# JosephCatrambone/aruco3

Measured on AMD Instinct MI355X. Metric: frames/sec at 1920x1080 ARUCO dict, higher is better.
Workload: dtype u8

## Files before the change

aruco3_amd/_lib.py:

```python
import ctypes as C
from pathlib import Path

import numpy as np

import os

_HERE = Path(__file__).resolve().parent
LIB_PATH = Path(os.environ["A3_HIP_LIB"]).resolve() if os.environ.get("A3_HIP_LIB") else _HERE / "libaruco3_hip.so"

OK, ERR_INVALID, ERR_HIP, ERR_CAPACITY, ERR_INTERNAL, ERR_NO_DEVICE, ERR_LIMIT = 0, -1, -2, -3, -4, -5, -6
FMT_RGB8, FMT_RGBA8, FMT_L8, FMT_BGRA8 = 0, 1, 2, 3
FMT_YUYV8, FMT_UYVY8 = 5, 6
MEM_HOST, MEM_DEVICE = 0, 1
PROFILE_OFF, PROFILE_STAGES, PROFILE_THRESHOLD_ONLY, PROFILE_THRESHOLD_SAMPLED = 0, 1, 2, 3
STAGE_THRESHOLD, STAGE_CONTOUR, STAGE_DECODE = 0, 1, 2
STEP_WHOLE, STEP_DECODE_DEFERRED, STEP_HELD_RELEASED_BY_LAST, STEP_HELD_RELEASED_EARLY, STEP_BURST_LAST, STEP_HELD = 0, 1, 2, 3, 4, 5
REFINE_NONE, REFINE_SUBPIX, REFINE_EDGES = 0, 1, 2
BOARD_NONE, BOARD_OK = 0, 1
BOARD_MAX_MARKERS = 1024
DIST_NONE, DIST_RATIONAL = 0, 1
DIST_FISHEYE = 3
CHARUCO_MAX_CORNERS = 2048
CHARUCO_NO_ADJ = 0xFFFFFFFF
CALIB_FIX_PRINCIPAL_POINT, CALIB_ZERO_TANGENT_DIST, CALIB_FIX_K3, CALIB_RATIONAL_MODEL, CALIB_USE_INTRINSIC_GUESS = 1, 2, 4, 8, 16
CALIB_OK, CALIB_TOO_FEW, CALIB_NO_INIT, CALIB_NOT_FINITE = 1, 2, 3, 4
CALIB_VIEW_USED, CALIB_VIEW_TOO_FEW_POINTS, CALIB_VIEW_DEGENERATE = 1, 2, 3
CALIB_MAX_POINTS, CALIB_MAX_VIEWS, CALIB_MAX_CAMERAS, CALIB_MAX_CALL_VIEWS = 4096, 4096, 1024, 65536
FISHEYE_FIX_PRINCIPAL_POINT, FISHEYE_FIX_K1, FISHEYE_FIX_K2, FISHEYE_FIX_K3, FISHEYE_FIX_K4, FISHEYE_USE_INTRINSIC_GUESS = 1, 2, 4, 8, 16, 32
FISHEYE_START_MAX_R = 4.0
RIG_USE_EXTRINSIC_GUESS, RIG_FIX_EXTRINSICS = 1, 2
RIG_OK, RIG_NOT_CONNECTED, RIG_NOT_FINITE = 1, 2, 3
RIG_OBS_USED, RIG_OBS_TOO_FEW_POINTS, RIG_OBS_DEGENERATE = 1, 2, 3
RIG_FRAME_USED, RIG_FRAME_UNUSED = 1, 2
RIG_MAX_CAMERAS, RIG_MAX_FRAMES, RIG_MAX_RIGS, RIG_MAX_CALL_FRAMES, RIG_MAX_CALL_OBSERVATIONS = 8, 4096, 1024, 65536, 262144
HANDEYE_USE_GUESS, HANDEYE_FIX_X = 1, 2
HANDEYE_OK, HANDEYE_TOO_FEW_FRAMES, HANDEYE_NO_MOTION, HANDEYE_NOT_FINITE = 1, 2, 3, 4
HANDEYE_FRAME_USED, HANDEYE_FRAME_TOO_FEW_POINTS, HANDEYE_FRAME_DEGENERATE = 1, 2, 3
HANDEYE_MAX_FRAMES, HANDEYE_MAX_PROBLEMS, HANDEYE_MAX_CALL_FRAMES = 256, 1024, 65536
HANDEYE_MIN_PIVOT_RATIO = 1e-4
MAP_USE_GUESS, MAP_FIX_MAP = 1, 2
MAP_OK, MAP_NOT_CONNECTED, MAP_NOT_FINITE = 1, 2, 3
MAP_MARKER_USED, MAP_MARKER_UNSEEN, MAP_MARKER_UNREACHED = 1, 2, 3
MAP_FRAME_USED, MAP_FRAME_UNUSED = 1, 2
MAP_OBS_USED, MAP_OBS_DEGENERATE, MAP_OBS_UNREACHED = 1, 2, 3
MAP_MAX_MARKERS, MAP_MAX_FRAMES, MAP_MAX_MAPS, MAP_MAX_CALL_FRAMES, MAP_MAX_CALL_OBSERVATIONS, MAP_START_OBSERVATIONS = 128, 4096, 1024, 65536, 262144, 8
STEP_NAMES = {0: "whole", 1: "decode_deferred", 2: "held_released_by_last", 3: "held_released_early", 4: "burst_last", 5: "held"}

SYMBOLS = [
    "a3_abi_version", "a3_default_config", "a3_create", "a3_destroy", "a3_last_error", "a3_set_stream", "a3_get_stream", "a3_set_pool_limits",
    "a3_get_tau", "a3_order_after", "a3_set_debug_taps", "a3_detect_batch", "a3_detect_batch_pose", "a3_detect_batch_submit", "a3_detect_batch_collect", "a3_detect_batch_pose_submit", "a3_detect_batch_pose_collect",
    "a3_host_alloc", "a3_host_free", "a3_host_register", "a3_host_unregister", "a3_get_stats", "a3_synth_render", "a3_download_grey", "a3_download_thresholded",
    "a3_candidate_count", "a3_download_candidates", "a3_download_homographies", "a3_estimate_pose", "a3_estimate_pose_normalized",
    "a3_find_nearest", "a3_calculate_tau", "a3_set_profiling", "a3_get_profile",
    "a3_contour_count", "a3_download_contours", "a3_detection_record_bytes", "a3_pack_detections",
    "a3_default_refine_config", "a3_set_corner_refinement", "a3_get_refined_corners", "a3_refine_corners",
    "a3_set_board", "a3_get_board_poses", "a3_estimate_board_pose",
    "a3_default_recover_config", "a3_set_board_recovery", "a3_get_board_recovery", "a3_get_recovered_counts", "a3_recover_markers",
    "a3_default_distortion", "a3_set_distortion", "a3_get_undistorted_corners", "a3_undistort_points",
    "a3_default_charuco_config", "a3_set_charuco", "a3_get_charuco_corners", "a3_get_charuco_poses", "a3_interpolate_charuco",
    "a3_calibrate_cameras", "a3_calibrate_fisheye_cameras", "a3_calibrate_rigs", "a3_calibrate_hand_eyes", "a3_build_marker_maps",
    "a3_default_rectify", "a3_rectify_frames", "a3_set_rectification", "a3_get_rectification",
    "a3_reduce_frames", "a3_set_reduction", "a3_get_reduction",
]
CAND_DTYPE = np.dtype([("start_key", "<u4"), ("xy", "<u2", (8,))])
PROJ_DTYPE = np.dtype([("inv", "<f4", (9,)), ("ok", "<i4")])
CONTOUR_DTYPE = np.dtype([("frame", "<u4"), ("start_key", "<u4"), ("point_base", "<u4"), ("n", "<u4")])
INTERNAL_SYMBOLS = ["a3_debug_set_overlap", "a3_debug_build_flags", "a3_debug_spin", "a3_debug_set_hold", "a3_debug_set_jump_rounds", "a3_debug_launch_threshold", "a3_debug_kernel_time", "a3_selftest_ieee", "a3_debug_clockwise", "a3_debug_rotate_bits", "a3_debug_discard_too_near", "a3_debug_inject_candidates", "a3_debug_sample_frames", "a3_debug_frame_candidates", "a3_debug_contour_quads"]


class A3Error(RuntimeError):
    def __init__(self, code, message):
        super().__init__(f"aruco3_hip error {code}: {message}")
        self.code = code


class Config(C.Structure):
    _fields_ = [
        ("threshold_window", C.c_uint32),
        ("contour_simplification_epsilon", C.c_double),
        ("min_side_length_factor", C.c_float),
        ("min_corner_separation_factor", C.c_float),
        ("homography_sample_size", C.c_uint32),
        ("filter_high_bit_errors", C.c_uint8),
    ]


class MarkerRec(C.Structure):
    _fields_ = [
        ("frame", C.c_uint32),
        ("id", C.c_uint32),
        ("code", C.c_uint64),
        ("corners", C.c_uint32 * 8),
        ("hamming_distance", C.c_uint8),
        ("rotation", C.c_uint8),
        ("candidate_index", C.c_uint16),
    ]


MARKER_DTYPE = np.dtype([("frame", "<u4"), ("id", "<u4"), ("code", "<u8"), ("corners", "<u4", (8,)), ("hamming_distance", "u1"),
                         ("rotation", "u1"), ("candidate_index", "<u2")], align=True)
assert MARKER_DTYPE.itemsize == C.sizeof(MarkerRec) == 56


class PoseRec(C.Structure):
    _fields_ = [("error", C.c_float), ("rotation", C.c_float * 9), ("translation", C.c_float * 3)]


class Intrinsics(C.Structure):
    _fields_ = [("image_width", C.c_uint32), ("image_height", C.c_uint32), ("focal_x", C.c_float), ("focal_y", C.c_float),
                ("principal_x", C.c_float), ("principal_y", C.c_float)]


class RefineConfig(C.Structure):
    _fields_ = [("method", C.c_uint32), ("win_half", C.c_uint32), ("relative_win", C.c_float), ("max_iterations", C.c_uint32),
                ("min_shift", C.c_float)]


class BoardPoseRec(C.Structure):
    _fields_ = [("status", C.c_uint32), ("markers_used", C.c_uint32), ("markers_rejected", C.c_uint32), ("iterations", C.c_uint32),
                ("rms_px", C.c_float), ("alt_rms_px", C.c_float), ("rotation", C.c_float * 9), ("translation", C.c_float * 3)]


class RecoverConfig(C.Structure):
    _fields_ = [("mode", C.c_uint32), ("min_markers", C.c_uint32), ("max_distance_px", C.c_float), ("max_hamming", C.c_uint8),
                ("reserved", C.c_uint8 * 3)]


RECOVER_NO_BITS = 255


class DistortionRec(C.Structure):
    _fields_ = [("model", C.c_uint32), ("iterations", C.c_uint32), ("k1", C.c_float), ("k2", C.c_float), ("p1", C.c_float),
                ("p2", C.c_float), ("k3", C.c_float), ("k4", C.c_float), ("k5", C.c_float), ("k6", C.c_float),
                ("max_residual_px", C.c_float)]


class CharucoConfig(C.Structure):
    _fields_ = [("min_markers", C.c_uint32), ("refine", C.c_uint32), ("win_half", C.c_uint32), ("relative_win", C.c_float),
                ("max_iterations", C.c_uint32), ("min_shift", C.c_float)]


CHARUCO_CORNER_DTYPE = np.dtype([("frame", "<u4"), ("id", "<u4"), ("x", "<f4"), ("y", "<f4"), ("interp_x", "<f4"), ("interp_y", "<f4"),
                                 ("markers_used", "<u4"), ("window", "<u4")])
CHARUCO_POSE_DTYPE = np.dtype([("status", "<u4"), ("corners_used", "<u4"), ("iterations", "<u4"), ("reserved", "<u4"), ("rms_px", "<f4"),
                               ("alt_rms_px", "<f4"), ("rotation", "<f4", (9,)), ("translation", "<f4", (3,))])
BOARD_POSE_DTYPE = np.dtype([("status", "<u4"), ("markers_used", "<u4"), ("markers_rejected", "<u4"), ("iterations", "<u4"),
                             ("rms_px", "<f4"), ("alt_rms_px", "<f4"), ("rotation", "<f4", (9,)), ("translation", "<f4", (3,))])


class CalibCamera(C.Structure):
# ... 123 lines not shown
    def as_dict(self):
        d = {k: int(getattr(self, k)) for k, _ in self._fields_}
        d["released_others"] = (d["stepping"] >> 8) & 0xFF
        d["reruns"] = (d["stepping"] >> 16) & 0xFF
        d["stepping"] = STEP_NAMES.get(d["stepping"] & 0xFF, d["stepping"] & 0xFF)
        return d


_lib = None


def load():
    global _lib
    if _lib is not None:
        return _lib
    try:
        import torch
    except ImportError:
        pass
    if not LIB_PATH.exists():
        raise ImportError(f"{LIB_PATH} is missing: build the HIP library first (python -c 'import __graft_entry__ as g; g.build()'). "
                          "aruco3_amd has no CPU fallback.")
    L = C.CDLL(str(LIB_PATH))
    vp, u8p, u32p, u64p, f32p, f64p = C.c_void_p, C.POINTER(C.c_uint8), C.POINTER(C.c_uint32), C.POINTER(C.c_uint64), C.POINTER(C.c_float), C.POINTER(C.c_double)
    L.a3_abi_version.restype = C.c_int
    L.a3_default_config.restype = None
    L.a3_default_config.argtypes = [C.POINTER(Config)]
    L.a3_create.restype = C.c_int
    L.a3_create.argtypes = [C.c_int, C.POINTER(Config), u64p, C.c_size_t, C.c_uint8, C.c_uint8, C.POINTER(vp)]
    L.a3_destroy.restype = None
    L.a3_destroy.argtypes = [vp]
    L.a3_last_error.restype = C.c_char_p
    L.a3_last_error.argtypes = [vp]
    L.a3_set_stream.restype = C.c_int
    L.a3_set_stream.argtypes = [vp, vp]
    L.a3_get_stream.restype = C.c_int
    L.a3_get_stream.argtypes = [vp, C.POINTER(vp)]
    L.a3_detect_batch_pose_submit.restype = C.c_int
    L.a3_detect_batch_pose_submit.argtypes = [vp, vp, C.c_int, C.c_int, C.c_uint32, C.c_uint32, C.c_size_t, C.c_size_t, C.c_uint32, C.c_float,
                                              C.POINTER(Intrinsics), C.c_size_t]
    L.a3_detect_batch_pose_collect.restype = C.c_int
    L.a3_detect_batch_pose_collect.argtypes = [vp, vp, vp, C.c_size_t, u32p, C.POINTER(C.c_size_t)]
    L.a3_order_after.restype = C.c_int
    L.a3_order_after.argtypes = [vp, vp]
    L.a3_host_alloc.restype = C.c_int
    L.a3_host_alloc.argtypes = [C.c_size_t, C.POINTER(vp)]
    L.a3_host_free.restype = C.c_int
    L.a3_host_free.argtypes = [vp]
    L.a3_host_register.restype = C.c_int
    L.a3_host_register.argtypes = [vp, C.c_size_t]
    L.a3_host_unregister.restype = C.c_int
    L.a3_host_unregister.argtypes = [vp]
    L.a3_set_pool_limits.restype = C.c_int
    L.a3_set_pool_limits.argtypes = [vp, C.c_uint64, C.c_uint64]
    L.a3_get_tau.restype = C.c_int
    L.a3_get_tau.argtypes = [vp, u8p]
    L.a3_set_debug_taps.restype = C.c_int
    L.a3_set_debug_taps.argtypes = [vp, C.c_int]
    L.a3_detect_batch.restype = C.c_int
    L.a3_detect_batch.argtypes = [vp, vp, C.c_int, C.c_int, C.c_uint32, C.c_uint32, C.c_size_t, C.c_size_t, C.c_uint32, vp, C.c_size_t, u32p,
                                  C.POINTER(C.c_size_t)]
    L.a3_detect_batch_submit.restype = C.c_int
    L.a3_detect_batch_submit.argtypes = [vp, vp, C.c_int, C.c_int, C.c_uint32, C.c_uint32, C.c_size_t, C.c_size_t, C.c_uint32, C.c_size_t]
    L.a3_detect_batch_collect.restype = C.c_int
    L.a3_detect_batch_collect.argtypes = [vp, vp, C.c_size_t, u32p, C.POINTER(C.c_size_t)]
    L.a3_detect_batch_pose.restype = C.c_int
    L.a3_detect_batch_pose.argtypes = [vp, vp, C.c_int, C.c_int, C.c_uint32, C.c_uint32, C.c_size_t, C.c_size_t, C.c_uint32, C.c_float,
                                       C.POINTER(Intrinsics), vp, vp, C.c_size_t, u32p, C.POINTER(C.c_size_t)]
    L.a3_synth_render.restype = C.c_int
    L.a3_synth_render.argtypes = [C.c_int, vp, vp, C.c_uint32, vp, C.c_uint32, C.c_uint32, C.c_uint32, C.c_int, C.c_float, C.c_float, C.c_int,
                                  vp, C.c_size_t, C.c_size_t]
    if hasattr(L, "a3_debug_set_overlap"):
        L.a3_debug_set_overlap.restype = C.c_int
        L.a3_debug_set_overlap.argtypes = [C.c_int]
    if hasattr(L, "a3_debug_launch_threshold"):
        L.a3_debug_launch_threshold.restype = C.c_int
        L.a3_debug_launch_threshold.argtypes = [vp, vp, C.c_int, C.c_uint32, C.c_uint32, C.c_uint32]
    if hasattr(L, "a3_debug_set_hold"):
        L.a3_debug_set_hold.restype = C.c_int
        L.a3_debug_set_hold.argtypes = [C.c_int]
    if hasattr(L, "a3_debug_set_jump_rounds"):
        L.a3_debug_set_jump_rounds.restype = C.c_int
        L.a3_debug_set_jump_rounds.argtypes = [C.c_int]
    if hasattr(L, "a3_debug_spin"):
        L.a3_debug_spin.restype = C.c_int
        L.a3_debug_spin.argtypes = [vp, C.c_int, C.c_int, C.c_int]
    if hasattr(L, "a3_debug_build_flags"):
        L.a3_debug_build_flags.restype = C.c_int
        L.a3_debug_build_flags.argtypes = []
    L.a3_debug_kernel_time.restype = C.c_int
    L.a3_debug_kernel_time.argtypes = [vp, C.c_int, C.c_int, C.c_int, C.POINTER(C.c_float)]
    L.a3_get_stats.restype = C.c_int
    L.a3_get_stats.argtypes = [vp, C.POINTER(Stats)]
    L.a3_download_grey.restype = C.c_int
    L.a3_download_grey.argtypes = [vp, C.c_uint32, u8p]
    L.a3_download_thresholded.restype = C.c_int
    L.a3_download_thresholded.argtypes = [vp, C.c_uint32, u8p]
    L.a3_candidate_count.restype = C.c_int
    L.a3_candidate_count.argtypes = [vp, C.c_uint32, u32p, u32p]
    L.a3_download_candidates.restype = C.c_int
    L.a3_download_candidates.argtypes = [vp, C.c_uint32, C.c_int, u32p, C.c_size_t]
    L.a3_download_homographies.restype = C.c_int
    L.a3_download_homographies.argtypes = [vp, C.c_uint32, u8p, u8p, u64p, C.POINTER(C.c_int32), C.c_size_t]
    L.a3_estimate_pose.restype = C.c_int
    L.a3_estimate_pose.argtypes = [vp, u32p, C.c_size_t, C.c_float, C.POINTER(Intrinsics), C.c_uint32, C.c_uint32, C.POINTER(PoseRec)]
    L.a3_estimate_pose_normalized.restype = C.c_int
    L.a3_estimate_pose_normalized.argtypes = [vp, f32p, C.c_size_t, C.c_float, C.POINTER(PoseRec)]
    L.a3_find_nearest.restype = C.c_int
    L.a3_find_nearest.argtypes = [vp, u64p, C.c_size_t, u32p, u8p]
    L.a3_calculate_tau.restype = C.c_int
    L.a3_calculate_tau.argtypes = [C.c_int, u64p, C.c_size_t, u8p]
    L.a3_set_profiling.restype = C.c_int
    L.a3_set_profiling.argtypes = [vp, C.c_int]
    L.a3_get_profile.restype = C.c_int
    L.a3_get_profile.argtypes = [vp, C.c_int, f64p, u64p, C.c_int]
    L.a3_selftest_ieee.restype = C.c_int
    L.a3_selftest_ieee.argtypes = [vp, f64p, f64p, C.c_size_t, f64p, f64p, f32p, f32p]
    L.a3_contour_count.restype = C.c_int
    L.a3_contour_count.argtypes = [vp, C.c_uint32, u32p, u64p]
    L.a3_download_contours.restype = C.c_int
    L.a3_download_contours.argtypes = [vp, C.c_uint32, u32p, u32p, u32p, C.c_size_t, C.c_size_t]
    L.a3_detection_record_bytes.restype = C.c_size_t
    L.a3_detection_record_bytes.argtypes = [C.c_uint32, C.c_int]
    L.a3_pack_detections.restype = C.c_int
    L.a3_pack_detections.argtypes = [vp, C.c_uint32, C.c_uint32, C.c_int, vp, C.c_size_t]
    L.a3_debug_clockwise.restype = C.c_int
    L.a3_debug_clockwise.argtypes = [vp, C.POINTER(C.c_int32), C.c_size_t, C.POINTER(C.c_int32)]
    L.a3_debug_rotate_bits.restype = C.c_int
    L.a3_debug_rotate_bits.argtypes = [vp, u8p, C.c_uint32, C.c_uint32, u8p]
    L.a3_debug_inject_candidates.restype = C.c_int
    L.a3_debug_inject_candidates.argtypes = [vp, u32p, C.c_size_t]
    if hasattr(L, "a3_debug_sample_frames"):
        L.a3_debug_sample_frames.restype = C.c_int
        L.a3_debug_sample_frames.argtypes = [vp, C.c_int]
    if hasattr(L, "a3_refine_corners"):
        L.a3_default_refine_config.restype = None
        L.a3_default_refine_config.argtypes = [C.POINTER(RefineConfig)]
        L.a3_set_corner_refinement.restype = C.c_int
        L.a3_set_corner_refinement.argtypes = [vp, C.POINTER(RefineConfig)]
        L.a3_get_refined_corners.restype = C.c_int
        L.a3_get_refined_corners.argtypes = [vp, f32p, C.c_size_t, C.POINTER(C.c_size_t)]
        L.a3_refine_corners.restype = C.c_int
        L.a3_refine_corners.argtypes = [vp, vp, C.c_int, C.c_int, C.c_uint32, C.c_uint32, C.c_size_t, f32p, f32p, C.c_size_t]
    if hasattr(L, "a3_set_board"):
        L.a3_set_board.restype = C.c_int
        L.a3_set_board.argtypes = [vp, u32p, f32p, C.c_size_t]
        L.a3_get_board_poses.restype = C.c_int
        L.a3_get_board_poses.argtypes = [vp, vp, C.c_size_t, C.POINTER(C.c_size_t)]
        L.a3_estimate_board_pose.restype = C.c_int
        L.a3_estimate_board_pose.argtypes = [vp, u32p, f32p, C.c_size_t, C.POINTER(Intrinsics), C.c_uint32, C.c_uint32, C.POINTER(BoardPoseRec)]
    if hasattr(L, "a3_set_board_recovery"):
        u64p, u8p = C.POINTER(C.c_uint64), C.POINTER(C.c_uint8)
        L.a3_default_recover_config.restype = C.c_int
        L.a3_default_recover_config.argtypes = [vp, C.POINTER(RecoverConfig)]
        L.a3_set_board_recovery.restype = C.c_int
        L.a3_set_board_recovery.argtypes = [vp, C.POINTER(RecoverConfig)]
        L.a3_get_board_recovery.restype = C.c_int
        L.a3_get_board_recovery.argtypes = [vp, C.POINTER(RecoverConfig)]
        L.a3_get_recovered_counts.restype = C.c_int
        L.a3_get_recovered_counts.argtypes = [vp, u32p, C.c_size_t]
        L.a3_recover_markers.restype = C.c_int
        L.a3_recover_markers.argtypes = [vp, u32p, u32p, C.c_size_t, u32p, u64p, u8p, C.c_size_t, C.POINTER(RecoverConfig), vp, C.c_size_t,
                                         C.POINTER(C.c_size_t)]
    if hasattr(L, "a3_set_distortion"):
        L.a3_default_distortion.restype = None
        L.a3_default_distortion.argtypes = [C.POINTER(DistortionRec)]
# ... 675 lines not shown
```

aruco3_amd/csrc/a3_api.hip:

```cpp
#include <algorithm>
#include <atomic>
#include <cmath>
#include <chrono>
#include <cstddef>
#include <cstdio>
#include <cstring>
#include <mutex>
#include <string>
#include <vector>

#include "a3_common.h"
#include "a3_format.h"
#include "a3_internal.h"
#include "a3_launch.h"
#include "a3_readback.h"
#include "a3_rectify_check.h"
#include "a3_reduce_check.h"
#include "a3_solve_check.h"

using namespace a3;

namespace {

thread_local std::string g_create_error;

constexpr uint32_t kPatchCapMin = 32768, kPatchCapMax = 1u << 20;

struct DevBuf {
    void* p = nullptr;
    size_t cap = 0;
    hipError_t ensure(size_t bytes) {
        if (bytes <= cap) return hipSuccess;
        if (p) { hipError_t e = hipFree(p); p = nullptr; cap = 0; if (e != hipSuccess) return e; }
        hipError_t e = hipMalloc(&p, bytes);
        if (e == hipSuccess) cap = bytes;
        return e;
    }
    void release() { if (p) (void)hipFree(p); p = nullptr; cap = 0; }
    template <typename T> T* as() const { return reinterpret_cast<T*>(p); }
};

template <typename T> struct Seg { size_t off, n; };
struct Layout {
    DevBuf& buf;
    hipStream_t stream;
    size_t end = 0;
    template <typename T> Seg<T> add(size_t n, size_t elem = sizeof(T)) {
        const size_t off = (end + 255) & ~(size_t)255;
        end = off + n * elem;
        return {off, n};
    }
    hipError_t ensure() { return buf.ensure((end + 255) & ~(size_t)255); }
    template <typename T> T* at(Seg<T> s) const { return reinterpret_cast<T*>(buf.as<uint8_t>() + s.off); }
    template <typename T> hipError_t upload(Seg<T> s, const T* src, size_t n) const {
        return n ? hipMemcpyAsync(at(s), src, n * sizeof(T), hipMemcpyHostToDevice, stream) : hipSuccess;
    }
    template <typename T> hipError_t download(Seg<T> s, T* dst) const {
        return dst ? hipMemcpyAsync(dst, at(s), s.n * sizeof(T), hipMemcpyDeviceToHost, stream) : hipSuccess;
    }
    template <typename T> hipError_t zero_from(Seg<T> s) const { return hipMemsetAsync(at(s), 0, end - s.off, stream); }
};

struct Batch {
    const uint8_t* pixels = nullptr; int fmt = 0;
    uint32_t W = 0, H = 0, n = 0;
    size_t row_stride = 0, frame_stride = 0, out_cap = 0;
    bool want_pose = false, pose_has_intr = false;
    float pose_size_mm = 0.0f;
    a3_intrinsics pose_intr{};
    a3_refine_config refine{};
    bool refined = false;
    bool board = false;
    a3_distortion dist{};
    bool undist = false;
    bool charuco = false;
    a3_charuco_config charuco_cfg{};
    uint32_t charuco_nc = 0, charuco_guess = 0;
    bool recover = false;
    a3_recover_config recover_cfg{};
    uint32_t recover_slots = 0, recover_cap = 0;
    uint32_t sides = 0;
    bool has(int kind) const { return (sides >> kind & 1u) != 0; }
    enum class Plane { None, Rectified, Reduced } plane = Plane::None;
    PixelSrc frames{};
    uint32_t frames_W = 0, frames_H = 0;
    a3_rectify rect_r{};
    uint32_t reduce_f = 0;
    bool taps = false;
    bool sample_frames = false;
    int profiling = 0, profile_every = 1;
    int prof = 0;
    bool need_grey = false;
    bool grey_src = false;
    uint32_t max_cand = 0, patch_cap = 0, marker_cap = 0, guess = 0;
    bool active = false, device_plan = false;
    size_t n_chunks = 0;
    Readback rb;
    uint64_t chunk0_darts = 0;
    int rounds_max = 0;
    PixelSrc src{};
};

}

struct a3_ctx {
    int device = 0;
    hipStream_t own_stream = nullptr, stream = nullptr;
    hipEvent_t ev_in = nullptr;
    hipEvent_t ev_contours = nullptr, ev_k1 = nullptr, ev_k1_done = nullptr, ev_gate = nullptr;
    bool gates_declared = false;
    bool rest_held = false;
    int held_rc = 0;
    bool back_deferred = false;
    int back_rc = 0;
    bool allow_defer = false;
    int batch_mode = 0;
    std::atomic<uint32_t> stepping{0};
    uint32_t released_others = 0;
    uint32_t reruns = 0;
    a3_config cfg{};
    uint8_t num_bits = 0, tau = 0;
    uint32_t n_codes = 0, mark_size = 0;
    std::string err;

    uint64_t max_darts = kMaxDartsDefault;
    BatchHints hints;
    uint32_t dbg_nd = 0, dbg_frames = 0, dbg_chunks = 0;
    PixelSrc dbg_src{};
    std::vector<CandRec> inject;
    bool inject_armed = false;
    uint32_t inject_count = 0;
    Batch batch;
    bool pending_trivial = false;
    bool busy() const { return batch.active || pending_trivial; }
    bool debug_taps = false;
    bool debug_sample_frames = false;
    uint32_t patch_cap = 0;
    bool grey_valid = false;
    bool contours_valid = false;
    uint32_t tap_contours = 0; uint64_t tap_points = 0;
    bool markers_valid = false;
    uint32_t last_n = 0, last_max_per_frame = 0;
    int profiling = 0;
    int profile_every = 1;
    uint32_t batch_seq = 0;
    hipEvent_t ev[6] = {nullptr, nullptr, nullptr, nullptr, nullptr, nullptr};
    double prof_ms[A3_STAGE_COUNT] = {0, 0, 0};
    uint64_t prof_n[A3_STAGE_COUNT] = {0, 0, 0};
    a3_stats stats{};

    uint32_t W = 0, H = 0, frames = 0;

    DevBuf dict, in, grey, bin, frame_darts, frame_darts_dev, frame_base, pix_base, tile_darts;
    DevBuf d_xy, d_succ, fin, t_cur, t_next;
    DevBuf leader_list, leader_keep, entry_list, es_a, es_b;
    DevBuf contours, cyc_start_off, points;
    DevBuf cands, pre_xy, fin_xy, fin_count, work, outs, proj, patches, cand_big;
    DevBuf zero_blk;
    a3_marker* markers_ptr = nullptr;
    unsigned long long* frame_darts_ptr = nullptr;
    BatchScratch* head = nullptr; DeviceCounters* counters = nullptr; uint32_t* per_frame = nullptr; uint32_t* frame_cursor = nullptr; uint32_t* cand_count = nullptr;
    uint32_t last_marker_total = 0;
    DevBuf tmp_a, tmp_b, tmp_c, tmp_d;
    DevBuf hsum;
    DevBuf wtab;
    DevBuf pose_buf;
    void* side_dev[kSideKinds] = {};
    std::vector<uint8_t> side_h[kSideKinds];
    bool side_valid[kSideKinds] = {};
    a3_refine_config refine{};
    a3_refine_config refine_prm_cfg{};
    std::vector<float> refine_prm;
    DevBuf refined_buf;
    std::vector<uint32_t> board_ids;
    std::vector<uint8_t> board_slots;
    uint64_t board_version = 0, board_dev_version = 0;
    std::vector<uint16_t> board_slot_up;
    std::vector<uint8_t> board_slots_up;
    DevBuf board_slot_of, board_slot_rec, board_buf;
    a3_recover_config recover{};
    uint64_t recover_ids_version = 0;
    std::vector<uint32_t> recover_ids_up;
    DevBuf recover_ids, recover_counts, recover_det, recover_tmp;
    a3_distortion dist{};
    DevBuf undist_buf;
    a3_charuco_config charuco_cfg{};
    std::vector<uint32_t> charuco_tab_h;
    uint32_t charuco_nc = 0;
    uint64_t charuco_version = 0, charuco_dev_version = 0;
    std::vector<uint32_t> charuco_tab_up;
    a3_charuco_config charuco_prm_cfg{};
    std::vector<float> charuco_prm;
    DevBuf charuco_tab, charuco_tmp, charuco_buf, charuco_und, charuco_pose_buf;
    std::vector<a3_charuco_corner> h_charuco;
    bool charuco_valid = false;
    DevBuf solve_in, solve_scratch, solve_big, solve_out;
    DevBuf rect_in, rect_out;
    a3_rectify rect{};
    bool rect_on = false;
    a3_reduction reduction{};
    DevBuf plane;
    uint32_t last_charuco_total = 0;
    void* pinned = nullptr;
    size_t pinned_cap = 0;
    void* pinned_counts = nullptr;
    size_t pinned_counts_cap = 0;
    std::vector<uint32_t> h_cand_pre, h_cand_fin;
    bool counts_valid = false;
};

namespace {

int fail(a3_ctx* c, int code, const char* what, hipError_t e = hipSuccess) {
    char buf[512];
    if (e != hipSuccess) snprintf(buf, sizeof buf, "%s: %s", what, hipGetErrorString(e));
    else snprintf(buf, sizeof buf, "%s", what);
    if (c) c->err = buf; else g_create_error = buf;
    return code;
}

#define A3_HIP(call)                                                        \
    do {                                                                    \
        hipError_t e_ = (call);                                             \
        if (e_ != hipSuccess) return fail(ctx, A3_ERR_HIP, #call, e_);      \
    } while (0)

inline void spin_pause() {
#if defined(__x86_64__) || defined(__i386__)
    __builtin_ia32_pause();
#endif
}
constexpr auto kSpinBudget = std::chrono::milliseconds(2);

hipError_t wait_stream(hipStream_t st) {
    const auto t0 = std::chrono::steady_clock::now();
    for (;;) {
        const hipError_t e = hipStreamQuery(st);
        if (e != hipErrorNotReady) return e;
        if (std::chrono::steady_clock::now() - t0 > kSpinBudget) return hipStreamSynchronize(st);
        spin_pause();
    }
}

hipError_t wait_event(hipEvent_t ev, hipStream_t st) {
    (void)hipStreamQuery(st);
// ... 295 lines not shown
    const uint32_t n = b.n;
    const ZeroLayout z = zero_layout(1, n, n, b.marker_cap);
    A3_HIP(ctx->tile_darts.ensure(tile_darts_bytes(b.W, b.H, n)));
    A3_HIP(ctx->zero_blk.ensure(z.total));
    if (ctx->frame_darts_dev.cap < (size_t)n * 8) {
        A3_HIP(ctx->frame_darts_dev.ensure((size_t)n * 8));
        A3_HIP(hipMemsetAsync(ctx->frame_darts_dev.p, 0, ctx->frame_darts_dev.cap, st));
    }
    A3_HIP(ctx->frame_base.ensure((size_t)(n + 1) * 4));
    if (int rc = ensure_dart_pool(ctx, pool_darts_of(ctx->max_darts, cap_d, 1))) return rc;
    A3_HIP(ctx->pix_base.ensure((size_t)n * b.W * b.H * 4));
    A3_HIP(ctx->contours.ensure((size_t)ctx->hints.max_contours * sizeof(ContourRec)));
    A3_HIP(ctx->cyc_start_off.ensure((size_t)ctx->hints.max_contours * 4));
    A3_HIP(ctx->points.ensure(ctx->hints.max_points * 4));
    return ensure_back_buffers(ctx, b, z.head_bytes);
}


int enqueue_front(a3_ctx* ctx, Batch& b, bool held) {
    hipStream_t st = ctx->stream;
    const uint32_t n = b.n, W = b.W, H = b.H;
    const size_t npx = (size_t)W * H;
    const uint32_t kMaxCand = ctx->hints.max_cand;
    const bool big_window = threshold_writes_grey_plane(ctx->cfg.threshold_window);
    b.need_grey = b.taps || big_window;
    b.grey_src = big_window || (b.taps && !b.sample_frames);
    if (b.need_grey) A3_HIP(ctx->grey.ensure(npx * n));
    ctx->grey_valid = b.need_grey;
    if (big_window) A3_HIP(ctx->hsum.ensure(npx * n * 2));
    const size_t bits_per_frame = (size_t)words_per_row(W) * 8 * H;
    A3_HIP(ctx->bin.ensure(bits_per_frame * n));
    A3_HIP(ctx->frame_darts.ensure((size_t)n * 8));
    A3_HIP(ctx->cands.ensure((size_t)n * kMaxCand * sizeof(CandRec)));
    A3_HIP(ctx->pre_xy.ensure((size_t)n * kMaxCand * 16));
    A3_HIP(ctx->fin_xy.ensure((size_t)n * kMaxCand * 16));
    A3_HIP(ctx->fin_count.ensure((size_t)n * 4));
    A3_HIP(ctx->work.ensure((size_t)n * kMaxCand * 4));
    if (kMaxCand > frame_cand_lds_slots()) A3_HIP(ctx->cand_big.ensure((size_t)n * kMaxCand * 4));
    A3_HIP(ctx->outs.ensure((size_t)n * kMaxCand * decode_out_bytes()));
    A3_HIP(ctx->proj.ensure((size_t)n * kMaxCand * proj_rec_bytes()));
    b.max_cand = kMaxCand;
    b.marker_cap = marker_cap_of(kMaxCand, n, b.out_cap);
    b.guess = marker_guess_of(ctx->last_marker_total, b.marker_cap);
    b.patch_cap = (uint32_t)std::min<uint64_t>(kPatchCapMax, std::max<uint64_t>(kPatchCapMin, (uint64_t)n * kMaxCand));
    if (b.taps) { A3_HIP(ctx->patches.ensure((size_t)b.patch_cap * ctx->cfg.homography_sample_size * ctx->cfg.homography_sample_size)); ctx->patch_cap = b.patch_cap; }
    ctx->W = W; ctx->H = H; ctx->frames = n;
    ctx->stats = a3_stats{};
    ctx->contours_valid = false; ctx->markers_valid = false; ctx->side_valid[kSidePoses] = false;

    b.prof = b.profiling == 1 && (ctx->batch_seq++ % (uint32_t)b.profile_every) != 0 ? 0 : b.profiling;
    const PixelSrc& fr = b.frames;
    if (b.plane == Batch::Plane::Rectified)
        A3_HIP(launch_rectify_grey(st, {.src = fr.base, .src_row = (size_t)fr.row_stride, .src_frame = (size_t)fr.frame_stride, .n_frames = n, .fmt = fr.fmt,
                                        .r = &b.rect_r, .grey = ctx->plane.as<uint8_t>()}));
    if (b.plane == Batch::Plane::Reduced)
        A3_HIP(launch_reduce_frames(st, {.src = fr.base, .src_row = (size_t)fr.row_stride, .src_frame = (size_t)fr.frame_stride, .n_frames = n, .fmt = fr.fmt,
                                         .W = b.frames_W, .H = b.frames_H, .factor = b.reduce_f, .dst = ctx->plane.as<uint8_t>(), .dst_row = W,
                                         .dst_frame = npx}));
    if (b.prof) A3_HIP(hipEventRecord(ctx->ev[0], st));
    A3_HIP(launch_grey_threshold(st, {.pixels = b.pixels, .fmt = b.fmt, .row_stride = b.row_stride, .frame_stride = b.frame_stride, .W = (int)W, .H = (int)H,
                                      .n = n, .radius = ctx->cfg.threshold_window, .grey = b.need_grey ? ctx->grey.as<uint8_t>() : nullptr,
                                      .bits = ctx->bin.as<uint64_t>(), .hsum_tmp = big_window ? ctx->hsum.as<uint16_t>() : nullptr}));
    if (b.prof) A3_HIP(hipEventRecord(ctx->ev[1], st));
    if (!held) return A3_OK;
    A3_HIP(hipEventRecord(ctx->ev_k1_done, st));
    const uint64_t cap_d = device_plan_capacity(ctx->hints, ctx->max_darts, n, W, H);
    if (cap_d == 0) return fail(ctx, A3_ERR_INTERNAL, "a chain was held back for a batch that needs a host-side plan");
    return ensure_chain_buffers(ctx, st, b, cap_d);
}

ContourChunk contour_chunk(const a3_ctx* ctx) {
    ContourChunk c;
    c.W = (int)ctx->W; c.H = (int)ctx->H; c.batch_frames = ctx->frames;
    c.bits = ctx->bin.as<uint64_t>(); c.tile_darts = ctx->tile_darts.as<uint32_t>(); c.pix_base = ctx->pix_base.as<uint32_t>();
    c.d_rec = ctx->d_xy.as<uint64_t>(); c.d_succ = ctx->d_succ.as<uint32_t>();
    c.entry_list = ctx->entry_list.as<uint32_t>(); c.es_a = ctx->es_a.p; c.es_b = ctx->es_b.p; c.fin = ctx->fin.p;
    c.leader_count = ctx->head->leader_count; c.entry_count = ctx->head->entry_count;
    c.leader_list = ctx->leader_list.as<uint32_t>(); c.leader_keep = ctx->leader_keep.as<uint32_t>();
    c.t_cur = ctx->t_cur.as<uint64_t>(); c.t_next = ctx->t_next.as<uint64_t>();
    c.contours = ctx->contours.as<ContourRec>(); c.cyc_start_off = ctx->cyc_start_off.as<uint32_t>(); c.points = ctx->points.as<uint32_t>();
    c.max_contours = ctx->hints.max_contours; c.max_points = ctx->hints.max_points;
    c.cands = ctx->cands.as<CandRec>(); c.cand_count = ctx->cand_count;
    c.err_flags = &ctx->head->err_flags;
    return c;
}

int enqueue_chain(a3_ctx* ctx, Batch& b, bool defer_locked) {
    hipStream_t st = ctx->stream;
    const uint32_t n = b.n, W = b.W, H = b.H;
    const int rel_mode = defer_locked ? 0 : release_mode();
    const size_t npx = (size_t)W * H;
    const uint32_t minwh = W < H ? W : H;
    const uint32_t min_edge_length = (uint32_t)((float)minwh * ctx->cfg.min_side_length_factor);
    const uint32_t kMaxCand = b.max_cand;
    bool released = false;
    auto release_waiting = [&]() -> int {
        if (released) return A3_OK;
        std::lock_guard<std::mutex> lk(g_defer_mu);
        bool any = false;
        for (a3_ctx* o : g_deferred) any |= (o != ctx && o->device == ctx->device);
        if (!any) return A3_OK;
        released = true;
        A3_HIP(hipEventRecord(ctx->ev_k1, st));
        const std::vector<a3_ctx*> list = g_deferred;
        for (a3_ctx* o : list)
            if (o != ctx && o->device == ctx->device)
                if (int rc = flush_deferred_locked(o, ctx->ev_k1)) { ctx->err = "deferred decode of another context: " + o->err; return rc; }
        return A3_OK;
    };
    if (rel_mode == 1) { if (int rc = release_waiting()) return rc; }

    const uint64_t cap_d = device_plan_capacity(ctx->hints, ctx->max_darts, n, W, H);
    const bool device_plan = cap_d != 0;
    size_t head_bytes = 0, head_off = 0;
    void* zero_p = nullptr; size_t zero_bytes = 0;
    auto layout_zero_block = [&](size_t n_chunks, uint32_t chunk_frames, bool launch) -> hipError_t {
        const ZeroLayout zl = zero_layout(n_chunks, chunk_frames, n, b.marker_cap);
        head_bytes = zl.head_bytes; head_off = zl.head_off;
        const hipError_t e = ctx->zero_blk.ensure(zl.total);
        if (e != hipSuccess) return e;
        uint8_t* z = ctx->zero_blk.as<uint8_t>();
        ctx->frame_cursor = reinterpret_cast<uint32_t*>(z);
        ctx->cand_count = ctx->frame_cursor + chunk_frames;
        ctx->head = reinterpret_cast<BatchScratch*>(z + head_off);
        ctx->counters = reinterpret_cast<DeviceCounters*>(ctx->head + 1);
        ctx->per_frame = reinterpret_cast<uint32_t*>(ctx->counters + n_chunks);
        ctx->markers_ptr = reinterpret_cast<a3_marker*>(z + head_off + head_bytes);
        zero_p = z; zero_bytes = (head_off + head_bytes + 15) & ~(size_t)15;
        return launch ? launch_zero(st, zero_p, zero_bytes) : hipSuccess;
    };
    std::vector<Chunk> chunks;
    std::vector<uint64_t> fd;
    if (device_plan) {
        if (int rc = ensure_chain_buffers(ctx, st, b, cap_d)) return rc;
        chunks.push_back(Chunk{0, n, cap_d, (uint32_t)std::min<uint64_t>(cap_d, 0xFFFFFFFFu)});
        A3_HIP(layout_zero_block(1, n, false));
        ctx->frame_darts_ptr = ctx->frame_darts_dev.as<unsigned long long>();
    } else {
        A3_HIP(ctx->tile_darts.ensure(tile_darts_bytes(W, H, n)));
        ctx->frame_darts_ptr = ctx->frame_darts.as<unsigned long long>();
        A3_HIP(hipMemsetAsync(ctx->frame_darts.p, 0, (size_t)n * 8, st));
    }
    DartCountLaunch count{.bits = ctx->bin.as<uint64_t>(), .W = (int)W, .H = (int)H, .n_frames = n, .frame_darts = ctx->frame_darts_ptr,
                          .tile_darts = ctx->tile_darts.as<uint32_t>(), .plan_cap = cap_d};
    if (device_plan) { count.frame_base = ctx->frame_base.as<uint32_t>(); count.plan = &ctx->head->plan; count.zero_p = zero_p; count.zero_bytes = zero_bytes; }
    A3_HIP(launch_dart_count(st, count));
    const uint32_t* n_live = device_plan ? &ctx->head->plan.darts : nullptr;
    uint32_t max_chunk_frames = n;
    if (!device_plan) {
        if (int rc = ensure_pinned(ctx, std::max<size_t>((size_t)n * 8, 1 << 16))) return rc;
        A3_HIP(hipMemcpyAsync(ctx->pinned, ctx->frame_darts.p, (size_t)n * 8, hipMemcpyDeviceToHost, st));
        A3_HIP(wait_stream(st));
        fd.assign((uint64_t*)ctx->pinned, (uint64_t*)ctx->pinned + n);
        chunks.resize(n);
        const ChunkSplit split = split_chunks(fd.data(), n, ctx->max_darts, kMaxChunkFrames, chunks.data());
        ctx->stats.darts += split.total_darts;
        if (split.refused) return fail(ctx, A3_ERR_LIMIT, "a frame needs more contour-graph nodes than 32-bit indices allow");
        ctx->max_darts = split.max_darts;
        chunks.resize(split.n_chunks);
        max_chunk_frames = split.max_chunk_frames;
        if (int rc = ensure_dart_pool(ctx, pool_darts_of(ctx->max_darts, split.max_chunk_darts, chunks.size()))) return rc;
        A3_HIP(ctx->pix_base.ensure((size_t)max_chunk_frames * npx * 4));
        A3_HIP(ctx->frame_base.ensure((size_t)(max_chunk_frames + 1) * 4 * chunks.size()));
        A3_HIP(layout_zero_block(chunks.size(), max_chunk_frames, true));
        A3_HIP(ctx->contours.ensure((size_t)ctx->hints.max_contours * sizeof(ContourRec)));
        A3_HIP(ctx->cyc_start_off.ensure((size_t)ctx->hints.max_contours * 4));
        A3_HIP(ctx->points.ensure(ctx->hints.max_points * 4));
        const size_t stride = max_chunk_frames + 1, n_bases = stride * chunks.size();
        if (int rc = ensure_pinned(ctx, (size_t)n * 8 + n_bases * 4 + (1 << 16))) return rc;
        uint32_t* h_bases = reinterpret_cast<uint32_t*>((uint8_t*)ctx->pinned + (size_t)n * 8);
        for (size_t ci = 0; ci < chunks.size(); ci++) chunk_frame_bases(fd.data(), chunks[ci], (uint32_t)stride, h_bases + ci * stride);
        A3_HIP(hipMemcpyAsync(ctx->frame_base.p, h_bases, n_bases * 4, hipMemcpyHostToDevice, st));
    }
    ctx->stats.chunks = (uint32_t)chunks.size();

    ContourChunk cc = contour_chunk(ctx);
    cc.n_live = n_live;
    cc.resolve_iters = ctx->hints.resolve_full_ttl > 0 ? ctx->hints.resolve_iters_hint : 0;
    cc.inline_resolve_W = ctx->hints.resolve_full_ttl > 0 ? 0 : (int)W;
    cc.min_edge_length = min_edge_length;
    cc.eps_factor = ctx->cfg.contour_simplification_epsilon;
    cc.keep_all = b.taps;
    cc.max_cand = kMaxCand;
    int rounds_max = 0;
    for (size_t ci = 0; ci < chunks.size(); ci++) {
        const Chunk& c = chunks[ci];
        const uint32_t nd = (uint32_t)c.darts;
        if (nd == 0) continue;
        if (ci > 0) {
            A3_HIP(hipMemsetAsync(cc.leader_count, 0, sizeof(BatchScratch::leader_count) + sizeof(BatchScratch::entry_count), st));
            A3_HIP(hipMemsetAsync(ctx->frame_cursor, 0, (size_t)c.count * 4, st));
        }
        cc.first_frame = c.first; cc.n_frames = c.count; cc.n_darts = nd;
        cc.frame_base = ctx->frame_base.as<uint32_t>() + ci * (max_chunk_frames + 1);
        cc.ctr = ctx->counters + ci;
        A3_HIP(launch_dart_build(st, cc));
        const int rounds = chunk_rounds(c.max_frame_darts, ctx->hints.jump_rounds_hint, g_jump_rounds_cap.load(std::memory_order_relaxed));
        rounds_max = std::max(rounds_max, rounds);
        cc.max_rounds = rounds;
        cc.frame_entries = ctx->hints.entry_global_ttl > 0 ? nullptr : ctx->frame_cursor;
        const bool dense_graph = (uint64_t)nd * 10u >= (uint64_t)c.count * npx;
        cc.dead_count = (b.taps || !dense_graph) ? nullptr : ctx->head->dead_count;
        cc.phase = 1;
        A3_HIP(launch_rank_cycles(st, cc));
        if (rel_mode == 2) { if (int rc = release_waiting()) return rc; }
        ctx->dbg_nd = nd; ctx->dbg_frames = c.count; ctx->dbg_chunks = (uint32_t)chunks.size();
        cc.phase = 2;
        A3_HIP(launch_rank_cycles(st, cc));
        A3_HIP(launch_resolve(st, cc));
        A3_HIP(launch_select_scatter(st, cc));
        A3_HIP(launch_contour_quads(st, cc));
    }
    if (rel_mode != 0) { if (int rc = release_waiting()) return rc; }
    if (b.prof >= 2) A3_HIP(hipEventRecord(ctx->ev[2], st));

    b.src = b.grey_src ? PixelSrc{ctx->grey.as<uint8_t>(), W, (unsigned long long)npx, kFmtGreyPlane}
                        : PixelSrc{b.pixels, b.row_stride, b.frame_stride, b.fmt};
    ctx->dbg_src = b.src;
    if (int rc = ensure_back_buffers(ctx, b, head_bytes)) return rc;
    b.device_plan = device_plan; b.n_chunks = chunks.size(); b.chunk0_darts = chunks.empty() ? 0 : chunks[0].darts;
    b.rounds_max = rounds_max;
    ctx->counts_valid = false;
    if (ctx->allow_defer && !defer_locked && b.profiling < 2 && ctx->batch_mode != 0) {
        A3_HIP(hipEventRecord(ctx->ev_contours, st));
        std::lock_guard<std::mutex> lk(g_defer_mu);
        ctx->back_deferred = true;
        ctx->back_rc = 0;
        ctx->stepping = A3_STEP_DECODE_DEFERRED;
        g_deferred.push_back(ctx);
    } else if (int rc = enqueue_back(ctx, st, b)) return rc;
    b.active = true;
    return A3_OK;
}

int enqueue_batch(a3_ctx* ctx) {
    ctx->stepping = A3_STEP_WHOLE;
    if (int rc = enqueue_front(ctx, ctx->batch, false)) return rc;
    return enqueue_chain(ctx, ctx->batch, false);
}

int finish_batch(a3_ctx* ctx, a3_marker* out, a3_pose* poses, size_t out_cap, uint32_t* per_frame_count, size_t* out_n) {
    Batch& b = ctx->batch;
    if (!b.active) return fail(ctx, A3_ERR_INVALID, "no batch was submitted");
    {
        std::lock_guard<std::mutex> lk(g_defer_mu);
        (void)flush_held_locked(ctx, nullptr);
        if (const int rc = ctx->held_rc) { ctx->held_rc = 0; b.active = false; return rc; }
    }
    b.active = false;
    hipStream_t st = ctx->stream;
    const size_t n_chunks = b.n_chunks;
    const uint32_t guess = b.guess, n = b.n;
    uint8_t* hp = (uint8_t*)ctx->pinned;
    Readback rb = b.rb;
    {
        std::lock_guard<std::mutex> lk(g_defer_mu);
        if (int rc = flush_deferred_locked(ctx, nullptr)) return rc;
        if (const int rc = ctx->back_rc) { ctx->back_rc = 0; return rc; }
    }
    A3_HIP(wait_event(ctx->ev[4], st));
    const BatchScratch& hs = *reinterpret_cast<const BatchScratch*>(hp);
    const DeviceCounters* hc = reinterpret_cast<const DeviceCounters*>(&hs + 1);
    const size_t slot_bytes = sizeof(CandRec) + 16 + 16 + 4 + decode_out_bytes() + proj_rec_bytes();
    const Verdict v = batch_verdict(hs, hc, {.n = n, .W = b.W, .H = b.H, .device_plan = b.device_plan, .n_chunks = n_chunks, .chunk0_darts = b.chunk0_darts,
                                             .rounds_max = b.rounds_max, .out_cap = out_cap, .lds_slots = frame_cand_lds_slots(), .slot_bytes = slot_bytes},
                                    ctx->hints);
    if (b.device_plan && !hs.plan.overflow) ctx->stats.darts = ctx->dbg_nd = v.darts;
    ctx->stats.contours_traced = v.contours_traced; ctx->stats.contours_materialised = v.contours_materialised;
    ctx->stats.jump_rounds = v.jump_rounds; ctx->stats.resolve_iterations = v.resolve_iterations;
    if (v.action == Verdict::Fail) return fail(ctx, v.code, v.message);
    if (v.action == Verdict::GrowCands) {
        const size_t had = ctx->cands.cap + ctx->pre_xy.cap + ctx->fin_xy.cap + ctx->work.cap + ctx->cand_big.cap + ctx->outs.cap + ctx->proj.cap;
        const size_t want = (size_t)n * v.next_cand * v.slot_bytes;
        size_t free_b = 0, total_b = 0;
        if (want > had && hipMemGetInfo(&free_b, &total_b) == hipSuccess && want - had > free_b)
            return fail(ctx, A3_ERR_LIMIT, "candidate tables of this batch do not fit the device (every frame gets the fullest frame's table): fewer frames per call");
        ctx->hints.max_cand = v.next_cand;
    }
    if (v.action != Verdict::Deliver) return 1;
    const uint32_t total = v.total, n_work = v.n_work, n_pre = v.n_pre;
    const uint32_t* hpf = reinterpret_cast<const uint32_t*>(hc + n_chunks);
    if (per_frame_count) memcpy(per_frame_count, hpf, (size_t)n * 4);
    uint32_t max_per_frame = 0;
    for (uint32_t f = 0; f < n; f++) max_per_frame = std::max(max_per_frame, hpf[f]);
    for (int k = 0; k < kSideKinds; k++)
        if (b.has(k) && kSides[k].per_frame) ctx->side_h[k].assign(at<uint8_t>(hp, rb.side[k]), at<uint8_t>(hp, rb.side[k]) + rb.side[k].bytes);
    if (b.charuco) {
        uint32_t charuco_total = 0;
        memcpy(&charuco_total, at<uint8_t>(hp, rb.charuco_total), 4);
        ctx->h_charuco.resize(charuco_total);
        const size_t staged = std::min<uint32_t>(charuco_total, b.charuco_guess);
        if (staged) memcpy(ctx->h_charuco.data(), at<uint8_t>(hp, rb.charuco), staged * sizeof(a3_charuco_corner));
        if (charuco_total > staged) {
            A3_HIP(hipMemcpyAsync(ctx->h_charuco.data() + staged, ctx->charuco_buf.as<a3_charuco_corner>() + staged,
                                  (charuco_total - staged) * sizeof(a3_charuco_corner), hipMemcpyDeviceToHost, st));
            A3_HIP(hipStreamSynchronize(ctx->stream));
        }
        ctx->last_charuco_total = charuco_total;
    }
    if (total > guess) {
        rb = refetch_layout(readback_shape(b, 0), total);
        if (int rc = ensure_pinned(ctx, pinned_bytes(rb))) return rc;
        hp = (uint8_t*)ctx->pinned;
        auto fetch = [&](const Span& to, const void* from) { return hipMemcpyAsync(at<uint8_t>(hp, to), from, to.bytes, hipMemcpyDeviceToHost, st); };
        A3_HIP(fetch(rb.markers, ctx->markers_ptr));
        for (int k = 0; k < kSideKinds; k++)
            if (b.has(k) && !kSides[k].per_frame) A3_HIP(fetch(rb.side[k], ctx->side_dev[k]));
        A3_HIP(hipStreamSynchronize(ctx->stream));
    }
    if (total) {
        memcpy(out, at<a3_marker>(hp, rb.markers), (size_t)total * sizeof(a3_marker));
        if (b.want_pose && poses) memcpy(poses, at<a3_pose>(hp, rb.side[kSidePoses]), (size_t)total * 2 * sizeof(a3_pose));
    }
    for (int k = 0; k < kSideKinds; k++) {
        const uint8_t* const h = at<uint8_t>(hp, rb.side[k]);
        if (b.has(k) && !kSides[k].per_frame && kSides[k].kept) ctx->side_h[k].assign(h, h + (size_t)total * kSides[k].rec);
        ctx->side_valid[k] = b.has(k);
    }
    ctx->charuco_valid = b.charuco;
    if (b.taps) {
        const uint32_t* hc32 = reinterpret_cast<const uint32_t*>(ctx->pinned_counts);
        ctx->h_cand_pre.assign(hc32, hc32 + n);
        ctx->h_cand_fin.assign(hc32 + n, hc32 + 2 * (size_t)n);
        for (auto& v : ctx->h_cand_pre) v = std::min(v, ctx->hints.max_cand);
        ctx->counts_valid = true;
    }
    ctx->last_marker_total = total;
    *out_n = total;
    ctx->stats.markers = total;
    ctx->stats.candidates = n_work;
    ctx->stats.candidates_pre = n_pre;
    ctx->markers_valid = true; ctx->last_n = n; ctx->last_max_per_frame = max_per_frame;
    ctx->contours_valid = b.taps && n_chunks == 1;
    if (ctx->contours_valid) { ctx->tap_contours = v.tap_contours; ctx->tap_points = v.tap_points; }
    if (b.prof >= 1) {
        float ms;
        A3_HIP(hipEventElapsedTime(&ms, ctx->ev[0], ctx->ev[1])); ctx->prof_ms[A3_STAGE_THRESHOLD] += ms; ctx->prof_n[A3_STAGE_THRESHOLD]++;
        if (b.prof >= 2) {
            A3_HIP(hipEventElapsedTime(&ms, ctx->ev[1], ctx->ev[2])); ctx->prof_ms[A3_STAGE_CONTOUR] += ms; ctx->prof_n[A3_STAGE_CONTOUR]++;
            A3_HIP(hipEventElapsedTime(&ms, ctx->ev[2], ctx->ev[3])); ctx->prof_ms[A3_STAGE_DECODE] += ms; ctx->prof_n[A3_STAGE_DECODE]++;
        }
    }
    return A3_OK;
}

int run_batch(a3_ctx* ctx, a3_marker* out, a3_pose* poses, size_t out_cap, uint32_t* per_frame_count, size_t* out_n) {
    if (int rc = enqueue_batch(ctx)) return rc;
    return finish_batch(ctx, out, poses, out_cap, per_frame_count, out_n);
}

// ... 534 lines not shown
        } else if (kernel == 1) {
            cc.dbg = dbg ? dbg : 5;
            A3_HIP(launch_dart_build(st, cc));
        } else if (kernel == 2) {
            cc.dbg = dbg ? dbg : 11;
            A3_HIP(launch_rank_cycles(st, cc));
        } else if (kernel == 3 || kernel == 4) {
            if (kernel == 4) {
                const size_t sweep = std::min<size_t>(ctx->pix_base.cap & ~(size_t)15, (size_t)512 << 20);
                if (sweep) A3_HIP(launch_zero(st, ctx->pix_base.p, sweep));
                A3_HIP(hipEventRecord(e0, st));
            }
            DecodeStage dec = decode_stage(ctx);
            dec.src = ctx->dbg_src; dec.W = cc.W; dec.H = cc.H; dec.max_cand = ctx->hints.max_cand; dec.few = ctx->frames <= 64u; dec.grid_blocks = 4096;
            dec.per_frame = nullptr;
            dec.projection = dbg >= 0; dec.variant = dbg < 0 ? -dbg : dbg;
            A3_HIP(launch_decode(st, dec));
        } else if (kernel == 6) {
            const Batch& b = ctx->batch;
            if (!b.refined || b.plane == Batch::Plane::Reduced || (dbg != A3_REFINE_SUBPIX && dbg != A3_REFINE_EDGES))
                return fail(ctx, A3_ERR_INVALID, "kernel 6: needs a preceding unreduced batch with corner refinement, and dbg = the method to time");
            a3_refine_config rc = b.refine;
            rc.method = (uint32_t)dbg;
            const RefineLaunch rl{.src = ctx->dbg_src, .W = (uint32_t)cc.W, .H = (uint32_t)cc.H, .markers = ctx->markers_ptr, .n_dev = &ctx->head->marker_total,
                                  .n = b.marker_cap, .params = refine_params_for(ctx, rc), .out = ctx->refined_buf.as<float>()};
            A3_HIP(dbg == A3_REFINE_EDGES ? launch_refine_edges(st, rl) : launch_refine_corners(st, rl));
        } else return fail(ctx, A3_ERR_INVALID, "kernel: 0 dart_count, 1 dart_assign, 2 local_contract, 3 decode, 4 decode on cold frames, 6 corner refinement");
        A3_HIP(hipEventRecord(e1, st));
        A3_HIP(hipStreamSynchronize(ctx->stream));
        float ms = 0;
        A3_HIP(hipEventElapsedTime(&ms, e0, e1));
        total += ms;
    }
    *avg_ms = (float)(total / reps);
    return A3_OK;
}

int a3_debug_set_overlap(int mode) {
    if (mode < -1 || mode > 2) return A3_ERR_INVALID;
    std::lock_guard<std::mutex> lk(g_defer_mu);
    if (!g_held.empty() || !g_deferred.empty()) return A3_ERR_INVALID;
    g_overlap_force.store(mode, std::memory_order_relaxed);
    return A3_OK;
}

int a3_debug_spin(void* hip_stream, int workgroups, int threads, int usec) {
    if (workgroups < 1 || workgroups > 1024 || threads < 64 || threads > 512 || threads % 64 || usec < 1 || usec > 100000) return A3_ERR_INVALID;
    static uint32_t* sink = nullptr;
    static std::mutex mu;
    {
        std::lock_guard<std::mutex> lk(mu);
        if (!sink) {
            if (hipMalloc(&sink, 4096 * 4) != hipSuccess) return A3_ERR_HIP;
            if (hipMemset(sink, 0, 4096 * 4) != hipSuccess) return A3_ERR_HIP;
        }
    }
    return launch_spin(reinterpret_cast<hipStream_t>(hip_stream), workgroups, threads, usec, sink) == hipSuccess ? A3_OK : A3_ERR_HIP;
}

int a3_debug_build_flags(void) { return 0; }

int a3_debug_launch_threshold(a3_ctx* ctx, const void* pixels_device, int fmt, uint32_t width, uint32_t height, uint32_t n_frames) {
    if (!ctx || !pixels_device || n_frames == 0) return A3_ERR_INVALID;
    A3_HIP(hipSetDevice(ctx->device));
    if (int rc = need_stream(ctx)) return rc;
    if (!format_valid(fmt) || format_width_error(fmt, width)) return A3_ERR_INVALID;
    const size_t bpp = format_bpp(fmt);
    if (threshold_writes_grey_plane(ctx->cfg.threshold_window))
        return fail(ctx, A3_ERR_INVALID, "a3_debug_launch_threshold: this threshold_window / frame layout takes the separable path, which needs a grey plane");
    A3_HIP(ctx->bin.ensure((size_t)words_per_row(width) * 8 * height * n_frames));
    A3_HIP(launch_grey_threshold(ctx->stream, {.pixels = reinterpret_cast<const uint8_t*>(pixels_device), .fmt = fmt, .row_stride = (size_t)width * bpp,
                                               .frame_stride = (size_t)width * bpp * height, .W = (int)width, .H = (int)height, .n = n_frames,
                                               .radius = ctx->cfg.threshold_window, .bits = ctx->bin.as<uint64_t>()}));
    return A3_OK;
}

int a3_debug_set_hold(int on) {
    std::lock_guard<std::mutex> lk(g_defer_mu);
    if (!g_held.empty()) return A3_ERR_INVALID;
    g_hold_rests = on != 0;
    return A3_OK;
}

int a3_debug_set_jump_rounds(int rounds) {
    if (rounds < 0 || rounds > 32) return A3_ERR_INVALID;
    g_jump_rounds_cap.store(rounds, std::memory_order_relaxed);
    return A3_OK;
}

int a3_synth_render(int device, void* hip_stream, const a3_synth_frame* frames, uint32_t n_frames, const a3_synth_marker* markers,
                    uint32_t n_markers, uint32_t width, uint32_t height, int paper, float black, float white, int supersample,
                    void* out_rgb_device, size_t row_stride, size_t frame_stride) {
    if (!frames || !out_rgb_device || (n_markers && !markers) || supersample < 1 || supersample > 8) return A3_ERR_INVALID;
    if (n_frames == 0 || width == 0 || height == 0) return A3_OK;
    if (row_stride == 0) row_stride = (size_t)width * 3;
    if (frame_stride == 0) frame_stride = row_stride * height;
    if (row_stride < (size_t)width * 3 || frame_stride < row_stride * (height - 1) + (size_t)width * 3 || height > 65535 || n_frames > 65535)
        return A3_ERR_INVALID;
    for (uint32_t f = 0; f < n_frames; f++)
        if ((uint64_t)frames[f].first_marker + frames[f].n_markers > n_markers) return A3_ERR_INVALID;
    for (uint32_t m = 0; m < n_markers; m++)
        if (markers[m].n == 0 || markers[m].n > 11) return A3_ERR_INVALID;
    if (hipSetDevice(device) != hipSuccess) return A3_ERR_NO_DEVICE;
    hipStream_t st = reinterpret_cast<hipStream_t>(hip_stream);
    a3_synth_frame* d_frames = nullptr; a3_synth_marker* d_markers = nullptr;
    hipError_t e = hipMalloc(&d_frames, sizeof(a3_synth_frame) * n_frames);
    if (e == hipSuccess && n_markers) e = hipMalloc(&d_markers, sizeof(a3_synth_marker) * n_markers);
    if (e == hipSuccess) e = hipMemcpyAsync(d_frames, frames, sizeof(a3_synth_frame) * n_frames, hipMemcpyHostToDevice, st);
    if (e == hipSuccess && n_markers) e = hipMemcpyAsync(d_markers, markers, sizeof(a3_synth_marker) * n_markers, hipMemcpyHostToDevice, st);
    if (e == hipSuccess) e = launch_synth_render(st, {.frames = d_frames, .n_frames = n_frames, .markers = d_markers, .W = width, .H = height, .paper = paper,
                                                      .black = black, .white = white, .supersample = supersample,
                                                      .out = reinterpret_cast<uint8_t*>(out_rgb_device), .row_stride = row_stride, .frame_stride = frame_stride});
    if (e == hipSuccess) e = hipStreamSynchronize(st);
    if (d_frames) (void)hipFree(d_frames);
    if (d_markers) (void)hipFree(d_markers);
    return e == hipSuccess ? A3_OK : A3_ERR_HIP;
}

int a3_get_stats(const a3_ctx* ctx, a3_stats* stats) {
    if (!ctx || !stats) return A3_ERR_INVALID;
    *stats = ctx->stats;
    stats->stepping = ctx->stepping | (std::min(ctx->released_others, 255u) << 8) | (std::min(ctx->reruns, 255u) << 16);
    return A3_OK;
}

static int download_plane(a3_ctx* ctx, const DevBuf& buf, uint32_t frame, uint8_t* dst) {
    if (!ctx || !dst) return A3_ERR_INVALID;
    if (frame >= ctx->frames) return fail(ctx, A3_ERR_INVALID, "frame index outside the last batch");
    const size_t npx = (size_t)ctx->W * ctx->H;
    A3_HIP(hipSetDevice(ctx->device));
    if (int rcs_ = need_stream(ctx)) return rcs_;
    A3_HIP(hipMemcpy(dst, buf.as<uint8_t>() + npx * frame, npx, hipMemcpyDeviceToHost));
    return A3_OK;
}

int a3_download_grey(a3_ctx* ctx, uint32_t frame, uint8_t* dst) {
    if (!ctx) return A3_ERR_INVALID;
    if (!ctx->grey_valid) return fail(ctx, A3_ERR_INVALID, "the grey plane is only kept when debug taps are enabled before the batch");
    return download_plane(ctx, ctx->grey, frame, dst);
}
int a3_download_thresholded(a3_ctx* ctx, uint32_t frame, uint8_t* dst) {
    if (!ctx || !dst) return A3_ERR_INVALID;
    if (frame >= ctx->frames) return fail(ctx, A3_ERR_INVALID, "frame index outside the last batch");
    const size_t npx = (size_t)ctx->W * ctx->H, wpf = (size_t)words_per_row(ctx->W) * ctx->H;
    A3_HIP(hipSetDevice(ctx->device));
    if (int rcs_ = need_stream(ctx)) return rcs_;
    A3_HIP(ctx->tmp_a.ensure(npx));
    A3_HIP(launch_unpack_bits(ctx->stream, ctx->bin.as<uint64_t>() + wpf * frame, (int)ctx->W, (int)ctx->H, ctx->tmp_a.as<uint8_t>()));
    A3_HIP(hipStreamSynchronize(ctx->stream));
    A3_HIP(hipMemcpy(dst, ctx->tmp_a.p, npx, hipMemcpyDeviceToHost));
    return A3_OK;
}

int a3_candidate_count(a3_ctx* ctx, uint32_t frame, uint32_t* n_pre, uint32_t* n_final) {
    if (!ctx) return A3_ERR_INVALID;
    if (frame >= ctx->frames) return fail(ctx, A3_ERR_INVALID, "frame index outside the last batch");
    if (ctx->counts_valid && frame < ctx->h_cand_fin.size()) {
        if (n_pre) *n_pre = ctx->h_cand_pre[frame];
        if (n_final) *n_final = ctx->h_cand_fin[frame];
        return A3_OK;
    }
    A3_HIP(hipSetDevice(ctx->device));
    if (int rcs_ = need_stream(ctx)) return rcs_;
    uint32_t a = 0, b = 0;
    A3_HIP(hipMemcpy(&a, ctx->cand_count + frame, 4, hipMemcpyDeviceToHost));
    A3_HIP(hipMemcpy(&b, ctx->fin_count.as<uint32_t>() + frame, 4, hipMemcpyDeviceToHost));
// ... 1110 lines not shown
```

aruco3_amd/csrc/a3_batch_head.h:

```cpp
#pragma once
#include <cstddef>
#include <cstdint>

#include "../../include/aruco3_hip.h"

namespace a3 {

template <typename T> constexpr T min_of(T a, T b) { return b < a ? b : a; }
template <typename T> constexpr T max_of(T a, T b) { return a < b ? b : a; }

constexpr uint32_t kMaxChunkFrames = 65536u;
constexpr int kResolveItersMax = 16;
constexpr uint32_t kLeaderShards = 16, kEntryShards = 16, kDeadShards = 16;

struct DeviceCounters {
    unsigned long long darts;
    unsigned long long points;
    unsigned int contours;
    unsigned int traced;
    unsigned int err_flags;
    unsigned int resolve_needed;
    unsigned int jump_changed[32];
    unsigned int resolve_changed[16];
    unsigned int entry_overflow;
    unsigned int pad[1];
};
static_assert(sizeof(DeviceCounters::resolve_changed) / sizeof(unsigned int) == kResolveItersMax, "one resolve_changed slot per pass");

constexpr unsigned kErrBrokenEvent = 1u,
                   kErrPointPool = 2u, kErrContourTable = 4u, kErrCandTable = 8u,
                   kErrResolve = 16u,
                   kErrMarkerCap = 32u,
                   kErrScatter = 64u;

struct PlanWords {
    uint32_t darts;
    uint32_t overflow;
    uint32_t max_frame_darts;
    uint32_t total_clamped;
};
struct BatchScratch {
    unsigned int work_count;
    unsigned int marker_total;
    unsigned int cand_pre_total;
    unsigned int pack_overflow;
    unsigned int err_flags;
    unsigned int cand_most;
    unsigned int unused6[2];
    PlanWords plan;
    unsigned int unused12[4];
    unsigned int leader_count[kLeaderShards];
    unsigned int entry_count[kEntryShards];
    unsigned int dead_count[kDeadShards];
};
static_assert(offsetof(BatchScratch, work_count) == 0 && offsetof(BatchScratch, marker_total) == 4 && offsetof(BatchScratch, cand_pre_total) == 8 &&
              offsetof(BatchScratch, pack_overflow) == 12 && offsetof(BatchScratch, err_flags) == 16 && offsetof(BatchScratch, cand_most) == 20 &&
              offsetof(BatchScratch, plan) == 32 && offsetof(PlanWords, darts) == 0 && offsetof(PlanWords, overflow) == 4 &&
              offsetof(PlanWords, max_frame_darts) == 8 && offsetof(PlanWords, total_clamped) == 12 && offsetof(BatchScratch, leader_count) == 64 &&
              offsetof(BatchScratch, entry_count) == 128 && offsetof(BatchScratch, dead_count) == 192 && sizeof(BatchScratch) == 256,
              "the scratch words' offsets are part of the read-back head");
static_assert(offsetof(BatchScratch, entry_count) == offsetof(BatchScratch, leader_count) + sizeof(BatchScratch::leader_count),
              "leader and entry counts are cleared by one memset");
constexpr unsigned kCandMostFromPre = (offsetof(BatchScratch, cand_most) - offsetof(BatchScratch, cand_pre_total)) / sizeof(unsigned int);

constexpr uint32_t kMaxCandDefault = 1024, kMaxCandLimit = A3_MAX_CANDIDATES_PER_FRAME;
static_assert(kMaxCandLimit == 65536, "a3_marker.candidate_index is a uint16_t");
constexpr uint32_t kMaxContoursDefault = 1u << 20;
constexpr uint64_t kMaxDartsDefault = 48ull << 20;
constexpr uint64_t kMaxPointsDefault = 64ull << 20;
constexpr uint64_t kHardMaxDarts = (1ull << 30) - (1ull << 16);
constexpr uint64_t kHardMaxPoints = 3ull << 30;

struct BatchHints {
    int jump_rounds_hint = 10, resolve_iters_hint = 4;
    int resolve_full_ttl = 0;
    int entry_global_ttl = 0;
    bool plan_valid = false, force_host_plan = false;
    uint32_t plan_n = 0, plan_W = 0, plan_H = 0;
    uint64_t plan_darts = 0;
    uint64_t max_points = kMaxPointsDefault;
    uint32_t max_contours = kMaxContoursDefault;
    uint32_t max_cand = kMaxCandDefault;
};

struct BatchFacts {
    uint32_t n, W, H; bool device_plan; size_t n_chunks; uint64_t chunk0_darts; int rounds_max; size_t out_cap; uint32_t lds_slots; size_t slot_bytes;
};
struct Verdict {
    enum Action { Deliver, Rerun, GrowCands, Fail } action = Deliver;
    int code = A3_OK; const char* message = nullptr;
    uint32_t next_cand = 0; size_t slot_bytes = 0;
    uint64_t darts = 0, contours_traced = 0, contours_materialised = 0; uint32_t jump_rounds = 0, resolve_iterations = 0;
    uint32_t total = 0, n_work = 0, n_pre = 0;
    uint32_t tap_contours = 0; uint64_t tap_points = 0;
};

inline Verdict batch_verdict(const BatchScratch& hs, const DeviceCounters* hc, const BatchFacts& f, BatchHints& h) {
    Verdict v;
    const auto rerun = [&v]() { v.action = Verdict::Rerun; return v; };
    const auto fail = [&v](int code, const char* message) { v.action = Verdict::Fail; v.code = code; v.message = message; return v; };
    if (f.device_plan) {
        if (hs.plan.overflow) { h.force_host_plan = true; return rerun(); }
        v.darts = hs.plan.darts;
        h.plan_darts = hs.plan.darts;
    } else {
        h.plan_valid = f.n_chunks == 1;
        h.plan_n = f.n; h.plan_W = f.W; h.plan_H = f.H;
        h.plan_darts = f.n_chunks == 1 ? f.chunk0_darts : 0;
    }
    unsigned int flags = hs.err_flags;
    for (unsigned int dead : hs.dead_count) v.contours_traced += dead;
    uint64_t need_points = 0; uint32_t need_contours = 0;
    bool jump_short = false, resolve_needed = false, entry_overflow = false;
    for (size_t ci = 0; ci < f.n_chunks; ci++) {
        const DeviceCounters& c = hc[ci];
        flags |= c.err_flags;
        resolve_needed |= c.resolve_needed != 0;
        entry_overflow |= c.entry_overflow != 0;
        need_points = max_of<uint64_t>(need_points, c.points);
        need_contours = max_of(need_contours, c.contours);
        v.contours_traced += c.traced;
        v.contours_materialised += c.contours;
        for (int r = 0; r < 32; r++) if (c.jump_changed[r]) v.jump_rounds = max_of<uint32_t>(v.jump_rounds, r + 1);
        uint32_t it = c.resolve_needed ? 1 : 0;
        for (int r = 0; r < kResolveItersMax - 1; r++) if (c.resolve_changed[r]) it = r + 2;
        v.resolve_iterations = max_of(v.resolve_iterations, it);
        if (f.rounds_max > 0 && f.rounds_max < 32 && c.jump_changed[f.rounds_max - 1] != 0) jump_short = true;
    }
    if (entry_overflow) { h.entry_global_ttl = 64; h.jump_rounds_hint = max_of(h.jump_rounds_hint, 12); return rerun(); }
    if (h.entry_global_ttl > 0) h.entry_global_ttl--;
    if (jump_short && h.jump_rounds_hint < 32) { h.jump_rounds_hint = 32; return rerun(); }
// ... 104 lines not shown
```

aruco3_amd/csrc/a3_internal.h:

```cpp
#ifndef ARUCO3_HIP_INTERNAL_H
#define ARUCO3_HIP_INTERNAL_H

#include "../../include/aruco3_hip.h"

#ifdef __cplusplus
extern "C" {
#endif

int  a3_debug_kernel_time(a3_ctx *ctx, int kernel, int dbg, int reps, float *avg_ms);

int  a3_debug_set_overlap(int mode);

int  a3_debug_spin(void *hip_stream, int workgroups, int threads, int usec);

int  a3_debug_set_hold(int on);

int  a3_debug_set_jump_rounds(int rounds);

int  a3_debug_launch_threshold(a3_ctx *ctx, const void *pixels_device, int fmt, uint32_t width, uint32_t height, uint32_t n_frames);

int  a3_debug_build_flags(void);

int  a3_selftest_ieee(a3_ctx *ctx, const double *a, const double *b, size_t n, double *sqrt_a, double *a_div_b,
                      float *sqrtf_a, float *a_divf_b);

int  a3_debug_clockwise(a3_ctx *ctx, const int32_t *quads_xy, size_t n, int32_t *out_xy);
int  a3_debug_rotate_bits(a3_ctx *ctx, const uint8_t *bits, uint32_t n, uint32_t times, uint8_t *out);
int  a3_debug_inject_candidates(a3_ctx *ctx, const uint32_t *quads_xy, size_t n);
int  a3_debug_sample_frames(a3_ctx *ctx, int enabled);
int  a3_debug_discard_too_near(a3_ctx *ctx, const uint32_t *quads_xy, size_t n, float min_distance, uint32_t *out_xy, size_t *n_out);

typedef struct { uint32_t start_key; uint16_t xy[8]; } a3_debug_cand;
#define A3_DEBUG_PROJ_BYTES 40
int  a3_debug_frame_candidates(a3_ctx *ctx, uint32_t n_frames, uint32_t max_cand, const uint32_t *cand_count, const a3_debug_cand *records,
                               float min_distance, uint32_t S, uint16_t *pre_xy, uint16_t *fin_xy, uint32_t *fin_count, uint32_t *work,
                               uint32_t *work_count, void *proj);

typedef struct { uint32_t frame, start_key, point_base, n; } a3_debug_contour;
int  a3_debug_contour_quads(a3_ctx *ctx, uint32_t width, uint32_t height, uint32_t n_darts, double eps_factor, uint32_t min_edge_length,
                            uint32_t first_frame, uint32_t n_frames, uint32_t max_cand, uint32_t max_contours, uint32_t ctr_contours,
                            uint32_t ctr_err_flags, const a3_debug_contour *records, uint32_t n_records, const uint32_t *points, size_t n_points,
                            uint32_t *cand_count, a3_debug_cand *cands, uint32_t *err_flags);

#ifdef __cplusplus
}
#endif
#endif
```

aruco3_amd/csrc/a3_launch.h:

```cpp
#pragma once

#include "a3_common.h"

namespace a3 {

struct ThresholdLaunch {
    const uint8_t* pixels = nullptr; int fmt = 0; size_t row_stride = 0, frame_stride = 0; int W = 0, H = 0; uint32_t n = 0, radius = 0;
    uint8_t* grey = nullptr; uint64_t* bits = nullptr; uint16_t* hsum_tmp = nullptr;
};
hipError_t launch_grey_threshold(hipStream_t st, const ThresholdLaunch& t);
bool threshold_writes_grey_plane(uint32_t radius);
hipError_t launch_k1_r1(hipStream_t st, const ThresholdLaunch& t);
hipError_t launch_k1_r2(hipStream_t st, const ThresholdLaunch& t);
bool ring_kernel_applies(uint32_t radius);
hipError_t launch_ring_threshold(hipStream_t st, const ThresholdLaunch& t);

size_t tile_darts_bytes(uint32_t W, uint32_t H, uint32_t n_frames);
struct DartCountLaunch {
    const uint64_t* bits = nullptr; int W = 0, H = 0; uint32_t first_frame = 0, n_frames = 0; unsigned long long* frame_darts = nullptr;
    uint32_t* tile_darts = nullptr; uint64_t plan_cap = 0; uint32_t* frame_base = nullptr; PlanWords* plan = nullptr; void* zero_p = nullptr;
    size_t zero_bytes = 0;
};
hipError_t launch_dart_count(hipStream_t st, const DartCountLaunch& d);
hipError_t launch_zero(hipStream_t st, void* p, size_t bytes);

size_t entry_state_bytes();
size_t fin_state_bytes();
size_t entry_slots(uint32_t n_darts);
size_t leader_list_bytes(uint32_t n_darts);

struct ContourChunk {
    uint32_t first_frame = 0, n_frames = 0, n_darts = 0; const uint32_t* frame_base = nullptr; DeviceCounters* ctr = nullptr;
    int max_rounds = 0;
    uint32_t* frame_entries = nullptr;
    unsigned int* dead_count = nullptr;
    int W = 0, H = 0;
    uint32_t batch_frames = 0;
    const uint64_t* bits = nullptr; const uint32_t* tile_darts = nullptr;
    const uint32_t* n_live = nullptr;
    uint32_t* pix_base = nullptr; uint64_t* d_rec = nullptr; uint32_t* d_succ = nullptr; uint32_t* entry_list = nullptr;
    unsigned int* entry_count = nullptr, * leader_count = nullptr;
    void* es_a = nullptr, * es_b = nullptr;
    void* fin = nullptr;
    uint32_t* leader_list = nullptr, * leader_keep = nullptr; uint64_t* t_cur = nullptr, * t_next = nullptr;
    int resolve_iters = 0;
    int inline_resolve_W = 0;
    uint32_t min_edge_length = 0; double eps_factor = 0.0; ContourRec* contours = nullptr; uint32_t* cyc_start_off = nullptr;
    uint32_t* points = nullptr; uint32_t max_contours = 0; uint64_t max_points = 0;
    bool keep_all = false;
    CandRec* cands = nullptr;
    uint32_t* cand_count = nullptr; uint32_t max_cand = 0; unsigned int* err_flags = nullptr;
    int phase = 0, dbg = 0;
};
hipError_t launch_dart_build(hipStream_t st, const ContourChunk& c);
hipError_t launch_rank_cycles(hipStream_t st, const ContourChunk& c);
hipError_t launch_resolve(hipStream_t st, const ContourChunk& c);
hipError_t launch_select_scatter(hipStream_t st, const ContourChunk& c);
hipError_t launch_contour_quads(hipStream_t st, const ContourChunk& c);
hipError_t launch_debug_clockwise(hipStream_t st, const int32_t* in, uint32_t n, int32_t* out);
hipError_t launch_unpack_bits(hipStream_t st, const uint64_t* bits, int W, int H, uint8_t* out);

size_t decode_out_bytes();
size_t proj_rec_bytes();
size_t weight_table_bytes();
uint32_t frame_cand_lds_slots();
struct DecodeStage {
    uint32_t n_frames = 0, first_frame = 0, max_cand = 0;
    const CandRec* cands = nullptr; const uint32_t* cand_count = nullptr; float min_distance = 0.0f;
    uint16_t* pre_xy = nullptr, * fin_xy = nullptr; uint32_t* fin_count = nullptr, * work = nullptr; unsigned int* work_count = nullptr;
    uint32_t S = 0; void* proj = nullptr; float* big_scratch = nullptr;
    PixelSrc src{}; int W = 0, H = 0; uint32_t n = 0, max_taps = 0; const uint64_t* dict = nullptr; uint32_t n_codes = 0, tau = 0; int filter = 0;
    const float* wtab = nullptr; void* outs = nullptr; uint8_t* patches = nullptr; uint32_t patch_cap = 0; uint32_t* per_frame = nullptr;
    int grid_blocks = 0; bool few = false;
    bool projection = false; int variant = 0;
    a3_marker* markers = nullptr; uint32_t marker_cap = 0; unsigned int* marker_total = nullptr, * err_flags = nullptr, * cand_pre_total = nullptr;
};
hipError_t launch_frame_candidates(hipStream_t st, const DecodeStage& d);
hipError_t launch_decode(hipStream_t st, const DecodeStage& d);
hipError_t launch_compact_markers(hipStream_t st, const DecodeStage& d);
hipError_t launch_weight_table(hipStream_t st, uint32_t S, uint32_t n, uint32_t max_taps, float* wtab);
hipError_t launch_pack_detections(hipStream_t st, const a3_marker* markers, const a3_pose* poses, const uint32_t* per_frame, uint32_t n_frames,
                                  uint32_t first_frame_global, uint32_t maxm, void* dst, unsigned int* overflow);
hipError_t launch_debug_rotate_bits(hipStream_t st, const uint8_t* in, uint32_t n, uint32_t r, uint8_t* out);
hipError_t launch_gather_patches(hipStream_t st, const void* outs_frame, uint32_t n_cand, const uint8_t* patches, uint32_t patch_cap, uint32_t S2,
                                 uint8_t* dst, unsigned int* missing);
struct PoseLaunch {
    const uint32_t* corners = nullptr; uint32_t corner_stride = 0; const float* norm_pts = nullptr; uint32_t n = 0;
    const unsigned int* n_dev = nullptr; int mode = 0; float marker_size_mm = 0.0f, iw = 0.0f, ih = 0.0f, fx = 0.0f, fy = 0.0f, cx = 0.0f, cy = 0.0f;
    a3_pose* out = nullptr;
};
hipError_t launch_pose(hipStream_t st, const PoseLaunch& p);
hipError_t launch_find_nearest(hipStream_t st, const uint64_t* dict, uint32_t n_codes, const uint64_t* bits, uint32_t n, uint32_t* idx, uint8_t* dist);
hipError_t launch_calc_tau(hipStream_t st, const uint64_t* dict, uint32_t n_codes, unsigned int* tau);
hipError_t launch_selftest(hipStream_t st, const double* a, const double* b, uint32_t n, double* sq, double* dv, float* sqf, float* dvf);

struct MarkerSrc {
    const a3_marker* markers = nullptr; const unsigned int* n_dev = nullptr; const uint32_t* per_frame = nullptr; const float* corners = nullptr;
    const uint32_t* ids = nullptr; const float* pts = nullptr; uint32_t n = 0, n_frames = 0;
};
struct BoardTables {
    const uint16_t* slot_of = nullptr; uint32_t n_codes = 0; const void* slots = nullptr; const float* cxy = nullptr; const uint32_t* adj = nullptr;
    uint32_t nc = 0;
};

size_t refine_params_bytes();
void refine_params(void* out, const a3_refine_config& cfg, uint32_t cells);
struct RefineLaunch {
    PixelSrc src{}; uint32_t W = 0, H = 0; const a3_marker* markers = nullptr; const unsigned int* n_dev = nullptr;
    const float* pts = nullptr, * cell_px = nullptr; uint32_t n = 0;
    const void* params = nullptr;
    float* out = nullptr;
};
hipError_t launch_refine_corners(hipStream_t st, const RefineLaunch& r);

hipError_t launch_refine_edges(hipStream_t st, const RefineLaunch& r);

hipError_t launch_undistort_corners(hipStream_t st, const a3_marker* markers, const float* pts, const unsigned int* n_dev, uint32_t n,
                                    const a3_intrinsics& in, const a3_distortion& d, float* out_xy, float* out_res);

size_t board_slot_bytes();
void board_slot_from(const float xy[8], void* out);
struct BoardPoseLaunch {
// ... 94 lines not shown
```

aruco3_amd/csrc/k_contours.hip:

```cpp
#include <algorithm>
#include <cmath>

#include "a3_common.h"
#include "a3_launch.h"


namespace a3 {

constexpr int kFinB = 8;
constexpr int kScatB = 1;

struct Nb8 { uint64_t c; uint64_t n[8]; };

__device__ __forceinline__ uint64_t ldw(const uint64_t* __restrict__ img, int wpr, int H, int j, int y) {
    return (y >= 0 && y < H && j >= 0 && j < wpr) ? img[(size_t)y * wpr + j] : 0ull;
}

__device__ __forceinline__ void pdart_words(const Nb8& nb, uint64_t p[8]) {
#pragma unroll
    for (int k = 0; k < 8; k++) {
        uint64_t m = nb.c & nb.n[k] & ~nb.n[(k + 7) & 7];
        if ((k & 1) == 0) m &= ~nb.n[(k + 6) & 7];
        p[k] = m;
    }
}

__device__ __forceinline__ uint32_t block_excl_scan_256(uint32_t v, uint32_t* s_wave, uint32_t* total) {
    const int lane = threadIdx.x & 63, wave = threadIdx.x >> 6;
    uint32_t inc = v;
#define A3_DPP_ADD(CTRL, ROWMASK) inc += (uint32_t)__builtin_amdgcn_update_dpp(0, (int)inc, CTRL, ROWMASK, 0xF, false);
    A3_DPP_ADD(0x111, 0xF)
    A3_DPP_ADD(0x112, 0xF)
    A3_DPP_ADD(0x114, 0xF)
    A3_DPP_ADD(0x118, 0xF)
    A3_DPP_ADD(0x142, 0xA)
    A3_DPP_ADD(0x143, 0xC)
#undef A3_DPP_ADD
    if (lane == 63) s_wave[wave] = inc;
    __syncthreads();
    uint32_t base = 0, tot = 0;
#pragma unroll
    for (int w = 0; w < 4; w++) {
        const uint32_t t = s_wave[w];
        if (w < wave) base += t;
        tot += t;
    }
    *total = tot;
    return base + inc - v;
}

constexpr int kTileWords = 4, kTileRows = 64;
__host__ __device__ inline uint32_t dart_tiles_x(uint32_t W) { return (words_per_row(W) + kTileWords - 1) / kTileWords; }
__host__ __device__ inline uint32_t dart_tiles(uint32_t W, uint32_t H) { return dart_tiles_x(W) * ((H + kTileRows - 1) / kTileRows); }

__device__ __forceinline__ void tile_stage(const uint64_t* __restrict__ img, int W, int H, uint32_t tile, uint64_t (*s_t)[kTileWords + 2]) {
    const int wpr = (int)words_per_row((uint32_t)W);
    const int tx = tile % dart_tiles_x((uint32_t)W), ty = tile / dart_tiles_x((uint32_t)W);
    const int j0 = tx * kTileWords - 1, y0 = ty * kTileRows - 1;
    constexpr int kStage = (kTileRows + 2) * (kTileWords + 2);
    static_assert(kStage <= 512, "two words per lane");
    uint64_t v[2];
#pragma unroll
    for (int k = 0; k < 2; k++) {
        const int i = min((int)threadIdx.x + 256 * k, kStage - 1);
        const int r = i / (kTileWords + 2), c = i - r * (kTileWords + 2);
        const int jj = j0 + c, yy = y0 + r;
        const uint64_t w = img[(size_t)min(max(yy, 0), H - 1) * wpr + min(max(jj, 0), wpr - 1)];
        v[k] = w & (0ull - (uint64_t)(yy >= 0 && yy < H && jj >= 0 && jj < wpr));
    }
#pragma unroll
    for (int k = 0; k < 2; k++) {
        const int i = (int)threadIdx.x + 256 * k;
        if (i < kStage) (&s_t[0][0])[i] = v[k];
    }
}
__device__ __forceinline__ Nb8 tile_nb8(const uint64_t (*s_t)[kTileWords + 2], int rl, int jl) {
    Nb8 r;
    const uint64_t al = s_t[rl][jl], a = s_t[rl][jl + 1], ar = s_t[rl][jl + 2];
    const uint64_t cl = s_t[rl + 1][jl], c = s_t[rl + 1][jl + 1], cr = s_t[rl + 1][jl + 2];
    const uint64_t bl = s_t[rl + 2][jl], b = s_t[rl + 2][jl + 1], br = s_t[rl + 2][jl + 2];
    r.c = c;
    r.n[0] = (c << 1) | (cl >> 63);
    r.n[1] = (a << 1) | (al >> 63);
    r.n[2] = a;
    r.n[3] = (a >> 1) | (ar << 63);
    r.n[4] = (c >> 1) | (cr << 63);
    r.n[5] = (b >> 1) | (br << 63);
// ... 89 lines not shown
            const unsigned long long bal = __ballot(hot);
            if (bal) {
                if (hot) {
                    const uint32_t below = __builtin_amdgcn_mbcnt_hi((uint32_t)(bal >> 32), __builtin_amdgcn_mbcnt_lo((uint32_t)bal, 0u));
                    const uint32_t slot = (qtail + below) & (kQ - 1);
                    q_c[slot] = c; q_up[slot] = up.c; q_dn[slot] = dn.c;
                    q_meta[slot] = cur.lr | (up.lr << 2) | (dn.lr << 4) | lane_row0 | ((uint32_t)(r0 + u) << 16);
                }
                qtail += (uint32_t)__popcll(bal);
                if (qtail - qhead >= 64u) {
                    wave_sync();
                    work((qhead + (uint32_t)lane) & (kQ - 1));
                    qhead += 64u;
                    wave_sync();
                }
            }
            up = cur; cur = dn;
        }
#pragma unroll
        for (int u = 0; u < kAhead; u++) nxt[u] = ahead[u];
    }
    wave_sync();
    if ((uint32_t)lane < qtail - qhead) work((qhead + (uint32_t)lane) & (kQ - 1));
    __builtin_amdgcn_s_waitcnt(0);
    __builtin_amdgcn_wave_barrier();
    uint32_t total = 0;
    if (gl < kTilesPerGroup && ty < (int)tiles_y) {
        const uint32_t tx = (uint32_t)(cx * kTilesPerGroup + gl);
        if (tx < tiles_x) {
            total = s_tile[grp][gl];
            (blockIdx.z ? tile_darts_h1 + (size_t)(blockIdx.z - 1) * gridDim.y * (tiles_x * tiles_y) : tile_darts)[(size_t)(first_frame + f) * (tiles_x * tiles_y) + ty * tiles_x + tx] = total;
        }
    }
    if (gl >= 1 && gl <= kOwners && ((gl - 1) & (kTileWords - 1)) == 0 && ty < (int)tiles_y) {
        const uint32_t tx = (uint32_t)(cx * kTilesPerGroup + (gl - 1) / kTileWords);
        if (tx < tiles_x) tile_mask[((size_t)(first_frame + f) * (tiles_x * tiles_y) + ty * tiles_x + tx) * kCountHalves + blockIdx.z] = s_mask[grp][(gl - 1) / kTileWords];
    }
#define A3_DPP_ADD(CTRL, ROWMASK) total += (uint32_t)__builtin_amdgcn_update_dpp(0, (int)total, CTRL, ROWMASK, 0xF, false);
    A3_DPP_ADD(0x111, 0xF) A3_DPP_ADD(0x112, 0xF) A3_DPP_ADD(0x114, 0xF) A3_DPP_ADD(0x118, 0xF) A3_DPP_ADD(0x142, 0xA) A3_DPP_ADD(0x143, 0xC)
#undef A3_DPP_ADD
    if (lane == 63 && total) atomicAdd(&frame_darts[f], (unsigned long long)total);
}

__device__ void plan_frames(unsigned long long* __restrict__ frame_darts, uint32_t n_frames, unsigned long long cap,
                            uint32_t* __restrict__ frame_base, PlanWords* __restrict__ plan) {
    __shared__ unsigned long long s_pw[4];
    __shared__ unsigned long long s_run;
    __shared__ unsigned int s_max;
    const int lane = threadIdx.x & 63, wave = threadIdx.x >> 6;
    if (threadIdx.x == 0) { s_run = 0; s_max = 0; }
    __syncthreads();
    for (uint32_t base = 0; base < n_frames; base += 256) {
        const uint32_t i = base + threadIdx.x;
        const unsigned long long v = i < n_frames ? frame_darts[i] : 0ull;
        if (i < n_frames) frame_darts[i] = 0ull;
        unsigned long long inc = v;
#pragma unroll
        for (int o = 1; o < 64; o <<= 1) { const unsigned long long t = __shfl_up(inc, o); if (lane >= o) inc += t; }
        if (lane == 63) s_pw[wave] = inc;
        atomicMax(&s_max, (unsigned int)min(v, 0xFFFFFFFFull));
        __syncthreads();
        unsigned long long before = s_run, tot = 0;
        for (int w = 0; w < 4; w++) { const unsigned long long t = s_pw[w]; if (w < wave) before += t; tot += t; }
        if (i < n_frames) frame_base[i] = (uint32_t)min(before + inc - v, 0xFFFFFFFFull);
        __syncthreads();
        if (threadIdx.x == 0) s_run += tot;
        __syncthreads();
    }
    if (threadIdx.x == 0) {
        const unsigned long long total = s_run;
        const bool fits = total <= cap;
        frame_base[n_frames] = fits ? (uint32_t)total : 0u;
        plan->darts = fits ? (uint32_t)total : 0u;
        plan->overflow = fits ? 0u : 1u;
        plan->max_frame_darts = s_max;
        plan->total_clamped = (uint32_t)min(total, 0xFFFFFFFFull);
    }
}

__global__ __launch_bounds__(256) void k_tile_scan(uint32_t* __restrict__ tile_darts, const uint32_t* __restrict__ tile_darts_h1, uint32_t tiles, uint32_t first_frame,
                                                   uint32_t* __restrict__ tile_off, uint32_t n_frames,
                                                   unsigned long long* __restrict__ frame_darts, unsigned long long cap,
                                                   uint32_t* __restrict__ frame_base, PlanWords* __restrict__ plan,
                                                   uint4* __restrict__ zero_p, uint32_t zero_n16) {
    if (blockIdx.x == n_frames) {
        for (uint32_t i = threadIdx.x; i < zero_n16; i += 256) zero_p[i] = make_uint4(0u, 0u, 0u, 0u);
        __syncthreads();
        plan_frames(frame_darts, n_frames, cap, frame_base, plan);
        return;
    }
    __shared__ uint32_t s_wave[4];
    __shared__ uint32_t s_run;
    const size_t base = (size_t)(first_frame + blockIdx.x) * tiles;
    if (threadIdx.x == 0) s_run = 0;
    __syncthreads();
    for (uint32_t t0 = 0; t0 < tiles; t0 += 256) {
        const uint32_t t = t0 + threadIdx.x;
        uint32_t v = 0;
        if (t < tiles) {
            v = tile_darts[base + t];
#pragma unroll
            for (int z = 1; z < kCountHalves; z++) v += tile_darts_h1[(size_t)(z - 1) * n_frames * tiles + base + t];
        }
        if (t < tiles) tile_darts[base + t] = v;
        uint32_t total;
        const uint32_t excl = block_excl_scan_256(v, s_wave, &total);
        if (t < tiles) tile_off[base + t] = s_run + excl;
        __syncthreads();
        if (threadIdx.x == 0) s_run += total;
        __syncthreads();
    }
}

__device__ __forceinline__ uint32_t row3(uint64_t l, uint64_t c, uint64_t r, int i) {
    const uint64_t v = i == 0 ? ((c << 1) | (l >> 63)) : (c >> (i - 1));
    return ((uint32_t)v & 7u) | (i == 63 ? ((uint32_t)r & 1u) << 2 : 0u);
}
__device__ __forceinline__ uint32_t tile_F(const uint64_t (*s_t)[kTileWords + 2], int rl, int jl, int i) {
    const uint32_t* base = reinterpret_cast<const uint32_t*>(&s_t[0][0]);
    const int p1 = (jl + 1) * 64 + i - 1, d = p1 >> 5, sh = p1 & 31;
    constexpr int kRowDwords = 2 * (kTileWords + 2);
    uint32_t rows[3];
#pragma unroll
    for (int k = 0; k < 3; k++) {
        const uint32_t* r = base + (rl + k) * kRowDwords + d;
        rows[k] = __builtin_amdgcn_alignbit(r[1], r[0], (uint32_t)sh) & 7u;
    }
    const uint32_t top = rows[0], mid = rows[1], bot = rows[2];
    return (mid & 1u) | ((top & 7u) << 1) | ((mid & 4u) << 2) | ((bot & 4u) << 3) | ((bot & 2u) << 5) | ((bot & 1u) << 7);
}
__device__ __forceinline__ int select_bit(uint64_t m, uint32_t r) {
    uint32_t w = (uint32_t)m, c = (uint32_t)__popc(w), pos = 0;
    if (r >= c) { w = (uint32_t)(m >> 32); r -= c; pos = 32; }
    c = (uint32_t)__popc(w & 0xFFFFu); if (r >= c) { w >>= 16; r -= c; pos += 16; }
    c = (uint32_t)__popc(w & 0xFFu);   if (r >= c) { w >>= 8;  r -= c; pos += 8; }
    c = (uint32_t)__popc(w & 0xFu);    if (r >= c) { w >>= 4;  r -= c; pos += 4; }
    c = (uint32_t)__popc(w & 3u);      if (r >= c) { w >>= 2;  r -= c; pos += 2; }
    return (int)(pos + (r >= (w & 1u) ? 1u : 0u));
}
struct PixLut { uint16_t v[256]; };
constexpr PixLut make_pix_lut() {
    PixLut t{};
    for (uint32_t F = 0; F < 256; F++) {
        const uint32_t rot1 = ((F << 1) | (F >> 7)) & 0xFFu, rot2 = ((F << 2) | (F >> 6)) & 0xFFu;
        const uint32_t P = F & ~rot1 & (0xAAu | ~rot2) & 0xFFu;
        uint32_t kW = 15, kE = 15;
        if (!(F & 1u)) { kW = 0; for (uint32_t b = 0; b < 7; b++) if ((F >> 1) & (1u << b)) { kW = b + 1; break; } }
        if (!(F & 16u)) {
            const uint32_t rr = ((F >> 5) | (F << 3)) & 0xFFu;
            uint32_t first = 0;
            for (uint32_t b = 0; b < 8; b++) if (rr & (1u << b)) { first = b + 1; break; }
            kE = (5 + first - 1) & 7;
        }
        t.v[F] = (uint16_t)(P | (kW << 8) | (kE << 12));
    }
    return t;
}
__device__ __constant__ const PixLut kPixLut = make_pix_lut();

__device__ __forceinline__ int dir_dx(int k) { return (int)((0x1A90u >> (2 * k)) & 3u) - 1; }
__device__ __forceinline__ int dir_dy(int k) { return (int)((0xA901u >> (2 * k)) & 3u) - 1; }

__global__ __launch_bounds__(256) void k_dart_assign(const uint64_t* __restrict__ bits, int W, int H, uint32_t first_frame,
                                                     const uint32_t* __restrict__ frame_base, const uint32_t* __restrict__ tile_off,
                                                     uint32_t* __restrict__ pix_base, const uint32_t* __restrict__ tile_darts,
                                                     uint64_t* __restrict__ d_rec, uint32_t* __restrict__ d_succ,
                                                     const uint32_t* __restrict__ n_live, int dbg,
                                                     const unsigned long long* __restrict__ tile_mask, uint32_t tiles, uint32_t n_frames) {
    __shared__ uint32_t s_wave[4];
    __shared__ uint64_t s_t[kTileRows + 2][kTileWords + 2];
    __shared__ uint64_t s_nodes[256];
    __shared__ uint64_t s_c0[256], s_c1[256], s_c2[256];
    __shared__ uint32_t s_dbase[256];
    __shared__ uint32_t s_mark[512];
    __shared__ uint16_t s_nbk[256];
    __shared__ uint8_t s_wofrank[256], s_rank[256], s_fr[256];
    __shared__ uint32_t s_multi;
    __shared__ uint16_t s_lut[256];
    const int wpr = (int)words_per_row((uint32_t)W);
    const uint32_t n_wg = tiles * n_frames, chunk = (n_wg + 7u) >> 3, g = (blockIdx.x & 7u) * chunk + (blockIdx.x >> 3);
    if (g >= n_wg) return;
    const uint32_t f = g / tiles, tile = g - f * tiles;
    if (tile_darts[(size_t)(first_frame + f) * tiles + tile] == 0u) return;
    if (n_live && *n_live == 0u) return;
    const uint32_t dart0 = frame_base[f] + tile_off[(size_t)(first_frame + f) * tiles + tile];
    if (dbg == 1) return;
    __shared__ uint32_t s_cnt[256];
    const unsigned long long* tm = tile_mask + ((size_t)(first_frame + f) * tiles + tile) * kCountHalves;
    static_assert(kCountHalves == 4 && kTileWords == 4 && kTileRows == 64, "four 64-bit word masks per tile, four word columns of 64 rows");
    unsigned long long cm[4];
#pragma unroll
    for (int c = 0; c < 4; c++)
        cm[c] = ((tm[0] >> (16 * c)) & 0xFFFFull) | (((tm[1] >> (16 * c)) & 0xFFFFull) << 16) | (((tm[2] >> (16 * c)) & 0xFFFFull) << 32) | (((tm[3] >> (16 * c)) & 0xFFFFull) << 48);
    const unsigned long long m0 = cm[0], m1 = cm[1], m2 = cm[2], m3 = cm[3];
    tile_stage(bits + (size_t)(first_frame + f) * wpr * H, W, H, tile, s_t);
    s_cnt[threadIdx.x] = 0;
    s_mark[threadIdx.x] = 0; s_mark[256 + threadIdx.x] = 0;
    s_lut[threadIdx.x] = kPixLut.v[threadIdx.x];
    if (threadIdx.x == 0) s_multi = 0;
    __syncthreads();
    const uint32_t a0 = (uint32_t)__popcll(m0), a1 = a0 + (uint32_t)__popcll(m1), a2 = a1 + (uint32_t)__popcll(m2), n_act = a2 + (uint32_t)__popcll(m3);
    for (uint32_t k = threadIdx.x; k < n_act; k += 256) {
        const uint32_t part = (k >= a0) + (k >= a1) + (k >= a2);
        const unsigned long long mm = part == 0 ? m0 : (part == 1 ? m1 : (part == 2 ? m2 : m3));
        const uint32_t w = part * 64u + (uint32_t)select_bit(mm, k - (part == 0 ? 0u : (part == 1 ? a0 : (part == 2 ? a1 : a2))));
        const Nb8 nb = tile_nb8(s_t, (int)(w & 63u), (int)(w >> 6));
        uint64_t p[8];
        pdart_words(nb, p);
        uint64_t nodes = 0;
        uint32_t nd = 0;
#pragma unroll
        for (int q = 0; q < 8; q++) { nd += __popcll(p[q]); nodes |= p[q]; }
        const uint64_t s1 = p[0] ^ p[1] ^ p[2], k1 = (p[0] & p[1]) | (p[2] & (p[0] ^ p[1]));
        const uint64_t s2 = p[3] ^ p[4] ^ p[5], k2 = (p[3] & p[4]) | (p[5] & (p[3] ^ p[4]));
        const uint64_t s3 = p[6] ^ p[7], k3 = p[6] & p[7];
        const uint64_t k4 = (s1 & s2) | (s3 & (s1 ^ s2));
        const uint64_t t = k1 ^ k2 ^ k3, q1 = (k1 & k2) | (k3 & (k1 ^ k2));
        s_nodes[w] = nodes;
        const uint64_t c1 = t ^ k4, c2 = q1 | (t & k4);
        s_c0[w] = s1 ^ s2 ^ s3; s_c1[w] = c1; s_c2[w] = c2;
        if ((c1 | c2) != 0ull) s_multi = 1u;
        s_cnt[w] = nd | ((uint32_t)__popcll(nodes) << 17);
        s_wofrank[k] = (uint8_t)w; s_rank[w] = (uint8_t)k;
    }
    __syncthreads();
    uint32_t total_p;
    const uint32_t excl_p = block_excl_scan_256(s_cnt[threadIdx.x], s_wave, &total_p);
    const uint32_t excl_d = excl_p & 0x1FFFFu, excl_n = excl_p >> 17, total_n = total_p >> 17;
    s_dbase[threadIdx.x] = excl_d;
    {
        const uint32_t cw = s_cnt[threadIdx.x] >> 17;
        if (cw) {
            const uint32_t k = s_rank[threadIdx.x];
            s_nbk[k] = (uint16_t)excl_n;
            if (excl_n) atomicOr(&s_mark[(excl_n - 1u) >> 5], 1u << ((excl_n - 1u) & 31u));
            const uint32_t seg = (excl_n + 63u) >> 6;
            if ((seg << 6) < excl_n + cw) s_fr[seg] = (uint8_t)k;
        }
    }
    if (dbg == 2) return;
    __syncthreads();
    if (dbg == 3) return;
    const int tx = tile % dart_tiles_x((uint32_t)W), ty = tile / dart_tiles_x((uint32_t)W);
    uint32_t* pbf = pix_base + (size_t)f * W * H;
    const bool single = __builtin_amdgcn_readfirstlane((int)s_multi) == 0;
    for (uint32_t n = threadIdx.x; n < total_n; n += 256) {
        const uint32_t seg = n >> 6;
        const uint32_t marks_below = __builtin_amdgcn_mbcnt_hi(s_mark[2u * seg + 1u], __builtin_amdgcn_mbcnt_lo(s_mark[2u * seg], 0u));
        const uint32_t kr = (uint32_t)s_fr[seg] + marks_below;
        const uint32_t w = s_wofrank[kr], r = n - (uint32_t)s_nbk[kr];
        const uint64_t m = s_nodes[w];
        const int i = select_bit(m, r);
        const int jl = w >> 6, rl = w & 63;
        const int wj = tx * kTileWords + jl, wy = ty * kTileRows + rl;
        const uint32_t F = tile_F(s_t, rl, jl, i);
        const uint32_t lut = s_lut[F];
        uint32_t P = lut & 0xFFu;
        const uint64_t below = (1ull << i) - 1ull;
        const uint32_t off = single ? (uint32_t)__popcll(m & below)
                                    : (uint32_t)__popcll(s_c0[w] & below) + 2u * (uint32_t)__popcll(s_c1[w] & below) + 4u * (uint32_t)__popcll(s_c2[w] & below);
        const int x = 64 * wj + i;
        uint32_t cur = dart0 + s_dbase[w] + off;
        if ((i == 0 || i == 63 || rl == 0 || rl == kTileRows - 1) && dbg != 4) pbf[(size_t)wy * W + x] = cur;
        const int kW = x > 0 ? (int)((lut >> 8) & 15u) : 15, kE = x + 1 < W ? (int)(lut >> 12) : 15;
        const uint32_t xy = (uint32_t)x | ((uint32_t)wy << 16);
        while (P) {
            const int k = __ffs(P) - 1;
            P &= P - 1;
            const uint32_t info = (uint32_t)k | (k == kW ? kInfoW : 0u) | (k == kE ? kInfoE : 0u);
            if (dbg != 4) d_rec[cur] = dart_rec(xy, F, info, f);
            const uint32_t rr = ((F >> k) | (F << (8 - k))) & 0xFFu;
            const int ko = (k + (31 - __clz(rr))) & 7, kin = (ko + 4) & 7;
            const int lx = jl * 64 + i + dir_dx(ko), ly = rl + dir_dy(ko);
            uint32_t succ;
            if (lx >= 0 && lx < kTileWords * 64 && ly >= 0 && ly < kTileRows) {
                const int j2 = lx >> 6, i2 = lx & 63, w2 = j2 * kTileRows + ly;
                const uint32_t P2 = (uint32_t)s_lut[tile_F(s_t, ly, j2, i2)] & 0xFFu;
                succ = cur;
                if ((P2 >> kin) & 1u) {
                    const uint64_t below2 = (1ull << i2) - 1ull;
                    const uint32_t off2 = single ? (uint32_t)__popcll(s_nodes[w2] & below2)
                                                 : (uint32_t)__popcll(s_c0[w2] & below2) + 2u * (uint32_t)__popcll(s_c1[w2] & below2) +
                                                   4u * (uint32_t)__popcll(s_c2[w2] & below2);
                    succ = dart0 + s_dbase[w2] + off2 + (uint32_t)__popc(P2 & ((1u << kin) - 1u));
                }
            } else {
                succ = kNone;
            }
            if (dbg != 4 || succ == 0x12345678u) d_succ[cur] = succ;
            cur++;
        }
    }
}

__device__ __forceinline__ uint32_t pixel_F(const uint64_t* __restrict__ img, int wpr, int H, int x, int y) {
    const int j = x >> 6, i = x & 63;
    uint32_t rows[3];
#pragma unroll
    for (int dy = -1; dy <= 1; dy++) {
        const uint64_t c = ldw(img, wpr, H, j, y + dy);
        const uint64_t l = i == 0 ? ldw(img, wpr, H, j - 1, y + dy) : 0ull;
        const uint64_t r = i == 63 ? ldw(img, wpr, H, j + 1, y + dy) : 0ull;
        rows[dy + 1] = row3(l, c, r, i);
    }
    const uint32_t top = rows[0], mid = rows[1], bot = rows[2];
    return (mid & 1u) | ((top & 7u) << 1) | ((mid & 4u) << 2) | ((bot & 4u) << 3) | ((bot & 2u) << 5) | ((bot & 1u) << 7);
}

__device__ __forceinline__ uint32_t cross_tile_succ(uint32_t d, uint64_t rec, int W, int H, int wpr, uint32_t first_frame,
                                                    const uint32_t* __restrict__ pix_base, const uint64_t* __restrict__ bits) {
    const uint32_t f = rec_frame(rec);
    const uint64_t* img = bits + (size_t)(first_frame + f) * wpr * H;
    const uint32_t* pb = pix_base + (size_t)f * W * H;
    const uint32_t xy = rec_xy(rec);
    const int x = xy & 0xFFFF, y = xy >> 16;
    const uint32_t F = rec_F(rec);
    const int k = rec_info(rec) & 7;
    const uint32_t r = ((F >> k) | (F << (8 - k))) & 0xFFu;
    const int ko = (k + (31 - __clz(r))) & 7;
    const int nx = x + dir_dx(ko), ny = y + dir_dy(ko);
    const uint32_t tP = pdart_mask(pixel_F(img, wpr, H, nx, ny));
    const int kin = (ko + 4) & 7;
    return ((tP >> kin) & 1u) ? pb[(size_t)ny * W + nx] + __popc(tP & ((1u << kin) - 1u)) : d;
}

__global__ __launch_bounds__(256) void k_dart_link(int W, int H, uint32_t first_frame, const uint32_t* __restrict__ pix_base,
                                                   const uint64_t* __restrict__ bits, const uint64_t* __restrict__ d_rec,
                                                   uint32_t* __restrict__ d_succ, uint32_t n_darts, const uint32_t* __restrict__ n_live) {
    if (n_live) n_darts = min(n_darts, *n_live);
    const int wpr = (int)words_per_row((uint32_t)W);
    constexpr int B = 8;
    const uint32_t stride = gridDim.x * blockDim.x;
    const uint32_t lane = threadIdx.x & 63u;
    for (uint32_t w0 = blockIdx.x * blockDim.x + (threadIdx.x & ~63u); w0 < n_darts; w0 += B * stride) {
        uint32_t sv[B];
#pragma unroll
        for (int u = 0; u < B; u++) sv[u] = d_succ[min(w0 + lane + (uint32_t)u * stride, n_darts - 1u)];
        uint64_t m[B];
        uint32_t total = 0;
#pragma unroll
        for (int u = 0; u < B; u++) {
            m[u] = __ballot(w0 + lane + (uint32_t)u * stride < n_darts && sv[u] == kNone);
            total += (uint32_t)__popcll(m[u]);
        }
        for (uint32_t j = lane; j < total; j += 64u) {
            uint32_t acc = 0, r = 0, su = 0;
            uint64_t mm = 0;
#pragma unroll
            for (int u = 0; u < B; u++) {
                const uint32_t c = (uint32_t)__popcll(m[u]);
                if (j >= acc && j < acc + c) { mm = m[u]; r = j - acc; su = (uint32_t)u; }
                acc += c;
            }
            const uint32_t d = w0 + (uint32_t)select_bit(mm, r) + su * stride;
            d_succ[d] = cross_tile_succ(d, d_rec[d], W, H, wpr, first_frame, pix_base, bits);
        }
    }
}

constexpr int kLT = 2048;
constexpr int kLTFrame = 1024;
__host__ __device__ inline uint32_t leader_shard_cap(uint32_t n_darts) { return n_darts / kLeaderShards + n_darts / 64u + 262144u; }
__host__ __device__ inline uint32_t entry_shard_cap(uint32_t n_darts) {
    const uint32_t tiles = (n_darts + kLT - 1) / kLT;
    return ((tiles + kEntryShards - 1) / kEntryShards) * kLT;
}
struct EntrySpace {
    uint32_t cnt[kEntryShards], span, total;
    __device__ explicit EntrySpace(const unsigned int* __restrict__ entry_count) {
        uint32_t m = 0;
#pragma unroll
        for (uint32_t sh = 0; sh < kEntryShards; sh++) { cnt[sh] = entry_count[sh]; m = max(m, cnt[sh]); }
        span = max((m + 63u) & ~63u, 64u);
        total = span * kEntryShards;
// ... 884 lines not shown
            if (num == 0) continue;
            const uint32_t index = ~(uint32_t)best & 0x3FFFFFFFu;
            const double dn = (double)num, den = (double)((long long)la * la + (long long)lb * lb);
            const double lhs = dn * dn, rhs = eps * eps * den;
            bool far;
            if (lhs > rhs * (1.0 + 1e-9)) far = true;
            else if (lhs < rhs * (1.0 - 1e-9)) far = false;
            else far = dn / sqrt(den) > eps;
            if (far) {
                if (splits == 3) { reject = true; break; }
                kept[splits++] = index;
                seg_a[nseg] = a; seg_b[nseg] = index; nseg++;
                seg_a[nseg] = index; seg_b[nseg] = b; nseg++;
            }
        }
        if (reject || splits != 3) continue;
        if (lane != 0) continue;
        uint32_t k0 = kept[0], k1 = kept[1], k2 = kept[2], t;
        if (k0 > k1) { t = k0; k0 = k1; k1 = t; }
        if (k1 > k2) { t = k1; k1 = k2; k2 = t; }
        if (k0 > k1) { t = k0; k0 = k1; k1 = t; }
        const uint32_t idx[4] = {0u, k0, k1, k2};
        int q[8], hq[8];
        for (int i = 0; i < 4; i++) { const uint32_t p = P[idx[i]]; q[2 * i] = p & 0xFFFF; q[2 * i + 1] = p >> 16; }
        if (!hull4(q, hq)) continue;
        uint32_t cmin = min_edge_length + 1u;
        for (int i = 0; i < 4; i++) {
            const int j = (i + 1) & 3;
            const int dx = hq[2 * i] - hq[2 * j], dy = hq[2 * i + 1] - hq[2 * j + 1];
            const uint32_t d2 = (uint32_t)(dx * dx + dy * dy);
            cmin = d2 < cmin ? d2 : cmin;
        }
        if (cmin < min_edge_length) continue;
        enforce_clockwise(hq);
        const uint32_t fl = r.frame - first_frame;
        const uint32_t slot = atomicAdd(&cand_count[fl], 1u);
        if (slot >= max_cand) { atomicOr(err_flags, kErrCandTable); continue; }
        CandRec cr;
        cr.start_key = r.start_key;
        for (int i = 0; i < 8; i++) cr.xy[i] = (uint16_t)hq[i];
        cands[(size_t)fl * max_cand + slot] = cr;
    }
}

__global__ __launch_bounds__(256) void k_contour_quads(uint32_t blocks64, const ContourRec* __restrict__ contours, const DeviceCounters* __restrict__ ctr,
                                                       uint32_t max_contours, const uint32_t* __restrict__ points, double eps_factor,
                                                       uint32_t min_edge_length, uint32_t first_frame, uint32_t max_cand,
                                                       CandRec* __restrict__ cands, uint32_t* __restrict__ cand_count,
                                                       unsigned int* __restrict__ err_flags, int coords14) {
    if (blockIdx.x < blocks64)
        contour_quads_body<64>(blockIdx.x, blocks64, contours, ctr, max_contours, points, eps_factor, min_edge_length, first_frame, max_cand, cands,
                               cand_count, err_flags, coords14 != 0);
    else
        contour_quads_body<16>(blockIdx.x - blocks64, gridDim.x - blocks64, contours, ctr, max_contours, points, eps_factor, min_edge_length,
                               first_frame, max_cand, cands, cand_count, err_flags, coords14 != 0);
}

__global__ void k_unpack_bits(const uint64_t* __restrict__ bits, int W, int H, uint8_t* __restrict__ out) {
    const int x = blockIdx.x * blockDim.x + threadIdx.x, y = blockIdx.y;
    if (x >= W) return;
    const int wpr = (int)words_per_row((uint32_t)W);
    out[(size_t)y * W + x] = ((bits[(size_t)y * wpr + (x >> 6)] >> (x & 63)) & 1ull) ? 255 : 0;
}

constexpr int kFinBlocks = 1536;
static inline int blocks_for(uint64_t n, int per_block, int cap) {
    uint64_t b = (n + per_block - 1) / per_block;
    if (b < 1) b = 1;
    if (b > (uint64_t)cap) b = cap;
    return (int)b;
}

__global__ __launch_bounds__(256) void k_zero(uint4* __restrict__ p, uint32_t n16) {
    for (uint32_t i = blockIdx.x * blockDim.x + threadIdx.x; i < n16; i += gridDim.x * blockDim.x) p[i] = make_uint4(0u, 0u, 0u, 0u);
}
hipError_t launch_zero(hipStream_t st, void* p, size_t bytes) {
    const uint32_t n16 = (uint32_t)(bytes / 16);
    hipLaunchKernelGGL(k_zero, dim3(blocks_for(n16, 256, 256)), dim3(256), 0, st, reinterpret_cast<uint4*>(p), n16);
    return hipGetLastError();
}

static size_t tile_off_offset(uint32_t W, uint32_t H, uint32_t n_frames) { return (size_t)dart_tiles(W, H) * n_frames; }
static size_t tile_mask_offset_bytes(uint32_t W, uint32_t H, uint32_t n_frames) { return ((size_t)dart_tiles(W, H) * n_frames * 4 * (1 + kCountHalves) + 7) & ~(size_t)7; }
size_t tile_darts_bytes(uint32_t W, uint32_t H, uint32_t n_frames) { return tile_mask_offset_bytes(W, H, n_frames) + (size_t)dart_tiles(W, H) * n_frames * kCountHalves * 8; }

hipError_t launch_dart_count(hipStream_t st, const DartCountLaunch& d) {
    const uint64_t* const bits = d.bits; const int W = d.W, H = d.H; const uint32_t first_frame = d.first_frame, n_frames = d.n_frames;
    unsigned long long* const frame_darts = d.frame_darts; uint32_t* const tile_darts = d.tile_darts; PlanWords* const plan = d.plan;
    const uint32_t tiles_x = dart_tiles_x((uint32_t)W), tiles_y = ((uint32_t)H + kTileRows - 1) / kTileRows;
    const uint32_t wpr = words_per_row((uint32_t)W);
    uint32_t* h1 = tile_darts + (size_t)tiles_x * tiles_y * n_frames * 2;
    unsigned long long* tmask = reinterpret_cast<unsigned long long*>(reinterpret_cast<uint8_t*>(tile_darts) + tile_mask_offset_bytes((uint32_t)W, (uint32_t)H, n_frames));
    if (wpr <= 30)
        hipLaunchKernelGGL(k_dart_count<32>, dim3((tiles_y + 1) / 2, n_frames, kCountHalves), dim3(64), 0, st, bits, W, H, first_frame, frame_darts, tile_darts, h1, tmask);
    else
        hipLaunchKernelGGL(k_dart_count<64>, dim3(((wpr + kCountLanes - 1) / kCountLanes) * tiles_y, n_frames, kCountHalves), dim3(64), 0, st, bits, W, H, first_frame,
                           frame_darts, tile_darts, h1, tmask);
    hipLaunchKernelGGL(k_tile_scan, dim3(n_frames + (plan ? 1u : 0u)), dim3(256), 0, st, tile_darts, h1, tiles_x * tiles_y, first_frame,
                       tile_darts + (size_t)tiles_x * tiles_y * n_frames, n_frames, frame_darts, (unsigned long long)d.plan_cap, d.frame_base, plan,
                       reinterpret_cast<uint4*>(d.zero_p), (uint32_t)(d.zero_bytes / 16));
    return hipGetLastError();
}

hipError_t launch_dart_build(hipStream_t st, const ContourChunk& c) {
    const uint32_t tiles = dart_tiles((uint32_t)c.W, (uint32_t)c.H);
    const uint32_t* const tile_off = c.tile_darts + tile_off_offset((uint32_t)c.W, (uint32_t)c.H, c.batch_frames);
    const unsigned long long* const tile_mask = reinterpret_cast<const unsigned long long*>(
        reinterpret_cast<const uint8_t*>(c.tile_darts) + tile_mask_offset_bytes((uint32_t)c.W, (uint32_t)c.H, c.batch_frames));
    hipLaunchKernelGGL(k_dart_assign, dim3((tiles * c.n_frames + 7u) / 8u * 8u), dim3(256), 0, st, c.bits, c.W, c.H, c.first_frame, c.frame_base, tile_off,
                       c.pix_base, c.tile_darts, c.d_rec, c.d_succ, c.n_live, c.dbg, tile_mask, tiles, c.n_frames);
    if (c.dbg && c.dbg != 5) return hipGetLastError();
    hipLaunchKernelGGL(k_dart_link, dim3(blocks_for(c.n_darts, 256, 4096)), dim3(256), 0, st, c.W, c.H, c.first_frame, c.pix_base, c.bits, c.d_rec, c.d_succ,
                       c.n_darts, c.n_live);
    return hipGetLastError();
}

size_t entry_state_bytes() { return sizeof(EntryState); }
static bool finalize_inline(bool frame_entries, bool trust_natural) { return frame_entries && trust_natural; }
size_t fin_state_bytes() { return sizeof(FinState); }
size_t entry_slots(uint32_t n_darts) { return (size_t)entry_shard_cap(n_darts) * kEntryShards; }
size_t leader_list_bytes(uint32_t n_darts) { return (size_t)leader_shard_cap(n_darts) * kLeaderShards * 4; }

hipError_t launch_rank_cycles(hipStream_t st, const ContourChunk& c) {
    const uint32_t n_darts = c.n_darts, n_frames = c.n_frames, min_edge_length = c.min_edge_length; const int W = c.W, dbg = c.dbg, phase = c.phase;
    const uint64_t* const d_rec = c.d_rec; const uint32_t* const d_succ = c.d_succ, * const n_live = c.n_live, * const frame_base = c.frame_base;
    uint32_t* const entry_list = c.entry_list, * const leader_list = c.leader_list, * const frame_entries = c.frame_entries;
    unsigned int* const entry_count = c.entry_count, * const leader_count = c.leader_count, * const dead_count = c.dead_count;
    DeviceCounters* const ctr = c.ctr;
    const int trust_natural = c.inline_resolve_W > 0 ? 1 : 0;
    const uint32_t ecap = entry_shard_cap(n_darts);
    FinState* fin = reinterpret_cast<FinState*>(c.fin);
    const bool no_finalize = finalize_inline(frame_entries != nullptr, trust_natural != 0) && dbg == 0;
    uint32_t* const ll = no_finalize ? leader_list : nullptr;
    const uint32_t lcap = leader_shard_cap(n_darts);
    if (phase != 2) {
        if (frame_entries && !dead_count)
            hipLaunchKernelGGL((k_local_contract<kLTFrame, false>), dim3((n_darts + kLTFrame - 1) / kLTFrame), dim3(256), 0, st, n_darts, W, d_rec, d_succ, fin,
                               entry_list, entry_count, ecap, frame_base, frame_entries, n_live, dbg, min_edge_length, dead_count, trust_natural,
                               ll, leader_count, lcap);
        else if (frame_entries)
            hipLaunchKernelGGL((k_local_contract<kLTFrame, true>), dim3((n_darts + kLTFrame - 1) / kLTFrame), dim3(256), 0, st, n_darts, W, d_rec, d_succ, fin,
                               entry_list, entry_count, ecap, frame_base, frame_entries, n_live, dbg, min_edge_length, dead_count, trust_natural,
                               ll, leader_count, lcap);
        else
            hipLaunchKernelGGL((k_local_contract<kLT, true>), dim3((n_darts + kLT - 1) / kLT), dim3(256), 0, st, n_darts, W, d_rec, d_succ, fin,
                               entry_list, entry_count, ecap, frame_base, frame_entries, n_live, dbg, min_edge_length, dead_count, trust_natural,
                               ll, leader_count, lcap);
    }
    if (dbg || phase == 1) return hipGetLastError();
    EntryState* a = reinterpret_cast<EntryState*>(c.es_a);
    EntryState* b = reinterpret_cast<EntryState*>(c.es_b);
    if (frame_entries) {
        hipLaunchKernelGGL(k_entry_frame, dim3(n_frames), dim3(256), 0, st, entry_list, frame_entries, frame_base, fin, d_rec, W, a, ctr,
                           ll, leader_count, lcap);
        if (no_finalize) return hipGetLastError();
        const int fin_blocks = std::max(blocks_for(n_darts, 256, kFinBlocks), (int)(((uint64_t)n_darts + 256ull * 32 - 1) / (256ull * 32)));
        hipLaunchKernelGGL(k_jump_finalize, dim3(fin_blocks), dim3(256), 0, st, n_darts, a, fin,
                           leader_list, leader_count, leader_shard_cap(n_darts), n_live, ctr);
        return hipGetLastError();
    }
    const dim3 grid(blocks_for(n_darts / 16 + 1, 256, 1024)), block(256);
    hipLaunchKernelGGL(k_entry_init, grid, block, 0, st, entry_list, entry_count, fin, d_rec, W, a, ecap);
    for (int r = 0; r < c.max_rounds; r++) {
        hipLaunchKernelGGL(k_entry_jump, grid, block, 0, st, a, b, entry_count, ecap, r, ctr);
        EntryState* t = a; a = b; b = t;
    }
    const int fin_blocks = std::max(blocks_for(n_darts, 256, kFinBlocks), (int)(((uint64_t)n_darts + 256ull * 32 - 1) / (256ull * 32)));
    hipLaunchKernelGGL(k_jump_finalize, dim3(fin_blocks), block, 0, st, n_darts, a, fin,
                       leader_list, leader_count, leader_shard_cap(n_darts), n_live, ctr);
    return hipGetLastError();
}

hipError_t launch_resolve(hipStream_t st, const ContourChunk& c) {
    const uint32_t n_darts = c.n_darts; const int W = c.W, max_iters = c.resolve_iters;
    const uint64_t* const d_rec = c.d_rec; uint64_t* const t_cur = c.t_cur, * const t_next = c.t_next;
    const uint32_t* const leader_list = c.leader_list, * const n_live = c.n_live; const unsigned int* const leader_count = c.leader_count;
    DeviceCounters* const ctr = c.ctr;
    const FinState* fin = reinterpret_cast<const FinState*>(c.fin);
    if (max_iters <= 0) return hipSuccess;
    const dim3 grid(blocks_for(n_darts, 256, 4096)), block(256);
    hipLaunchKernelGGL(k_resolve_fast, dim3(blocks_for(n_darts / 16 + 1, 256, 1024)), block, 0, st, fin, leader_list, leader_count,
                       leader_shard_cap(n_darts), W, d_rec, t_cur, ctr);
    hipLaunchKernelGGL(k_resolve_init, grid, block, 0, st, fin, d_rec, W, n_darts, t_cur, t_next, ctr, n_live);
    for (int it = 0; it < max_iters; it++) {
        hipLaunchKernelGGL(k_resolve_eval, grid, block, 0, st, fin, n_darts, W, d_rec, t_cur, t_next, it, ctr, n_live);
        hipLaunchKernelGGL(k_resolve_commit, grid, block, 0, st, fin, n_darts, t_cur, t_next, it, it == max_iters - 1 ? 1 : 0, ctr, n_live);
    }
    return hipGetLastError();
}

hipError_t launch_select_scatter(hipStream_t st, const ContourChunk& c) {
    const uint32_t n_darts = c.n_darts;
    const double image_diag = std::sqrt((double)c.W * c.W + (double)c.H * c.H);
// ... 34 lines not shown
```

Before: 391,000.

## Compact live tiles per frame and size dart-assign grid from last batch

The tile scan kernel now also builds a compacted per-frame list of tiles that contain darts, plus a count. The dart-assign kernel walks that list instead of launching one workgroup per tile and exiting early on empty ones. The grid is sized from the previous batch's longest live list, recorded on device and stored on the host, and each block loops over extra tiles when the list is longer. This removes launch and early-exit overhead for mostly empty frames. The cost is an extra scan in the tile-scan kernel, a device max-reduction, and a serial loop in blocks when the live count grows between batches.

Measured after the change: 385,100. 1.5% lower.

```diff
diff --git a/aruco3_amd/_lib.py b/aruco3_amd/_lib.py
--- a/aruco3_amd/_lib.py
+++ b/aruco3_amd/_lib.py
@@ -65,7 +65,7 @@
 CAND_DTYPE = np.dtype([("start_key", "<u4"), ("xy", "<u2", (8,))])
 PROJ_DTYPE = np.dtype([("inv", "<f4", (9,)), ("ok", "<i4")])
 CONTOUR_DTYPE = np.dtype([("frame", "<u4"), ("start_key", "<u4"), ("point_base", "<u4"), ("n", "<u4")])
-INTERNAL_SYMBOLS = ["a3_debug_set_overlap", "a3_debug_build_flags", "a3_debug_spin", "a3_debug_set_hold", "a3_debug_set_jump_rounds", "a3_debug_launch_threshold", "a3_debug_kernel_time", "a3_selftest_ieee", "a3_debug_clockwise", "a3_debug_rotate_bits", "a3_debug_discard_too_near", "a3_debug_inject_candidates", "a3_debug_sample_frames", "a3_debug_frame_candidates", "a3_debug_contour_quads"]
+INTERNAL_SYMBOLS = ["a3_debug_set_overlap", "a3_debug_build_flags", "a3_debug_spin", "a3_debug_set_hold", "a3_debug_set_jump_rounds", "a3_debug_set_assign_grid", "a3_debug_launch_threshold", "a3_debug_kernel_time", "a3_selftest_ieee", "a3_debug_clockwise", "a3_debug_rotate_bits", "a3_debug_discard_too_near", "a3_debug_inject_candidates", "a3_debug_sample_frames", "a3_debug_frame_candidates", "a3_debug_contour_quads"]
 
 
 class A3Error(RuntimeError):
@@ -355,6 +355,9 @@
     if hasattr(L, "a3_debug_set_jump_rounds"):
         L.a3_debug_set_jump_rounds.restype = C.c_int
         L.a3_debug_set_jump_rounds.argtypes = [C.c_int]
+    if hasattr(L, "a3_debug_set_assign_grid"):
+        L.a3_debug_set_assign_grid.restype = C.c_int
+        L.a3_debug_set_assign_grid.argtypes = [C.c_void_p, C.c_uint32]
     if hasattr(L, "a3_debug_spin"):
         L.a3_debug_spin.restype = C.c_int
         L.a3_debug_spin.argtypes = [vp, C.c_int, C.c_int, C.c_int]
diff --git a/aruco3_amd/csrc/a3_api.hip b/aruco3_amd/csrc/a3_api.hip
--- a/aruco3_amd/csrc/a3_api.hip
+++ b/aruco3_amd/csrc/a3_api.hip
@@ -13,6 +13,7 @@
 #include "a3_format.h"
 #include "a3_internal.h"
 #include "a3_launch.h"
+#include "a3_live_tiles.h"
 #include "a3_readback.h"
 #include "a3_rectify_check.h"
 #include "a3_reduce_check.h"
@@ -161,6 +162,8 @@
     unsigned long long* frame_darts_ptr = nullptr;
     BatchScratch* head = nullptr; DeviceCounters* counters = nullptr; uint32_t* per_frame = nullptr; uint32_t* frame_cursor = nullptr; uint32_t* cand_count = nullptr;
     uint32_t last_marker_total = 0;
+    bool live_known = false; uint32_t live_longest = 0, live_n = 0, live_W = 0, live_H = 0;
+    uint32_t dbg_assign_grid = 0;
     DevBuf tmp_a, tmp_b, tmp_c, tmp_d;
     DevBuf hsum;
     DevBuf wtab;
@@ -622,6 +625,8 @@
     c.max_contours = ctx->hints.max_contours; c.max_points = ctx->hints.max_points;
     c.cands = ctx->cands.as<CandRec>(); c.cand_count = ctx->cand_count;
     c.err_flags = &ctx->head->err_flags;
+    const bool known = ctx->live_known && ctx->live_n == ctx->frames && ctx->live_W == ctx->W && ctx->live_H == ctx->H;
+    c.assign_rows = ctx->dbg_assign_grid ? assign_rows_of_blocks(ctx->dbg_assign_grid, ctx->frames) : assign_rows_want(known, ctx->live_longest);
     return c;
 }
 
@@ -716,6 +721,7 @@
 
     ContourChunk cc = contour_chunk(ctx);
     cc.n_live = n_live;
+    cc.longest_list = chunks.size() == 1 ? &ctx->head->longest_list : nullptr;
     cc.resolve_iters = ctx->hints.resolve_full_ttl > 0 ? ctx->hints.resolve_iters_hint : 0;
     cc.inline_resolve_W = ctx->hints.resolve_full_ttl > 0 ? 0 : (int)W;
     cc.min_edge_length = min_edge_length;
@@ -806,6 +812,8 @@
                                              .rounds_max = b.rounds_max, .out_cap = out_cap, .lds_slots = frame_cand_lds_slots(), .slot_bytes = slot_bytes},
                                     ctx->hints);
     if (b.device_plan && !hs.plan.overflow) ctx->stats.darts = ctx->dbg_nd = v.darts;
+    ctx->live_known = n_chunks == 1 && n <= kLiveMaxFrames;
+    ctx->live_longest = hs.longest_list; ctx->live_n = n; ctx->live_W = b.W; ctx->live_H = b.H;
     ctx->stats.contours_traced = v.contours_traced; ctx->stats.contours_materialised = v.contours_materialised;
     ctx->stats.jump_rounds = v.jump_rounds; ctx->stats.resolve_iterations = v.resolve_iterations;
     if (v.action == Verdict::Fail) return fail(ctx, v.code, v.message);
@@ -1506,6 +1514,12 @@
     return A3_OK;
 }
 
+int a3_debug_set_assign_grid(a3_ctx* ctx, uint32_t blocks) {
+    if (!ctx) return A3_ERR_INVALID;
+    ctx->dbg_assign_grid = blocks;
+    return A3_OK;
+}
+
 int a3_debug_set_jump_rounds(int rounds) {
     if (rounds < 0 || rounds > 32) return A3_ERR_INVALID;
     g_jump_rounds_cap.store(rounds, std::memory_order_relaxed);
diff --git a/aruco3_amd/csrc/a3_batch_head.h b/aruco3_amd/csrc/a3_batch_head.h
--- a/aruco3_amd/csrc/a3_batch_head.h
+++ b/aruco3_amd/csrc/a3_batch_head.h
@@ -46,7 +46,8 @@
     unsigned int pack_overflow;
     unsigned int err_flags;
     unsigned int cand_most;
-    unsigned int unused6[2];
+    unsigned int longest_list;
+    unsigned int unused7[1];
     PlanWords plan;
     unsigned int unused12[4];
     unsigned int leader_count[kLeaderShards];
diff --git a/aruco3_amd/csrc/a3_internal.h b/aruco3_amd/csrc/a3_internal.h
--- a/aruco3_amd/csrc/a3_internal.h
+++ b/aruco3_amd/csrc/a3_internal.h
@@ -16,6 +16,8 @@
 int  a3_debug_set_hold(int on);
 
 int  a3_debug_set_jump_rounds(int rounds);
+
+int  a3_debug_set_assign_grid(a3_ctx *ctx, uint32_t blocks);
 
 int  a3_debug_launch_threshold(a3_ctx *ctx, const void *pixels_device, int fmt, uint32_t width, uint32_t height, uint32_t n_frames);
 
diff --git a/aruco3_amd/csrc/a3_launch.h b/aruco3_amd/csrc/a3_launch.h
--- a/aruco3_amd/csrc/a3_launch.h
+++ b/aruco3_amd/csrc/a3_launch.h
@@ -38,6 +38,7 @@
     uint32_t batch_frames = 0;
     const uint64_t* bits = nullptr; const uint32_t* tile_darts = nullptr;
     const uint32_t* n_live = nullptr;
+    uint32_t assign_rows = 0; uint32_t* longest_list = nullptr;
     uint32_t* pix_base = nullptr; uint64_t* d_rec = nullptr; uint32_t* d_succ = nullptr; uint32_t* entry_list = nullptr;
     unsigned int* entry_count = nullptr, * leader_count = nullptr;
     void* es_a = nullptr, * es_b = nullptr;
diff --git a/aruco3_amd/csrc/a3_live_tiles.h b/aruco3_amd/csrc/a3_live_tiles.h
--- /dev/null
+++ b/aruco3_amd/csrc/a3_live_tiles.h
@@ -0,0 +1,32 @@
+#pragma once
+#include <cstdint>
+
+namespace a3 {
+
+constexpr uint32_t kAssignGridMin = 8;
+constexpr uint32_t kLiveMaxFrames = 2048;
+
+struct LiveSlot { uint32_t f, r; };
+constexpr LiveSlot live_slot(uint32_t block, uint32_t rows, uint32_t n_frames) {
+    const uint32_t n = rows * n_frames, per_xcd = (n + 7u) >> 3, g = (block & 7u) * per_xcd + (block >> 3);
+    if (g >= n || (block >> 3) >= per_xcd) return LiveSlot{n_frames, 0u};
+    return LiveSlot{g / rows, g % rows};
+}
+
+inline uint32_t assign_rows(uint32_t want, uint32_t tiles) {
+    return want == 0 || want > tiles ? (tiles ? tiles : 1u) : want;
+}
+inline uint32_t assign_rows_want(bool known, uint32_t last_longest) {
+    if (!known) return 0;
+    const uint64_t want = (uint64_t)last_longest + last_longest / 16u + 2u;
+    return (uint32_t)(want > 0x7FFFFFFFull ? 0x7FFFFFFFull : want);
+}
+inline uint32_t assign_rows_of_blocks(uint32_t blocks, uint32_t n_frames) {
+    return blocks == 0 ? 0u : (blocks / (n_frames ? n_frames : 1u) ? blocks / (n_frames ? n_frames : 1u) : 1u);
+}
+inline uint32_t assign_grid(uint32_t rows, uint32_t n_frames) {
+    const uint32_t g = (rows * n_frames + 7u) / 8u * 8u;
+    return g < kAssignGridMin ? kAssignGridMin : g;
+}
+
+}
diff --git a/aruco3_amd/csrc/k_contours.hip b/aruco3_amd/csrc/k_contours.hip
--- a/aruco3_amd/csrc/k_contours.hip
+++ b/aruco3_amd/csrc/k_contours.hip
@@ -3,6 +3,7 @@
 
 #include "a3_common.h"
 #include "a3_launch.h"
+#include "a3_live_tiles.h"
 
 
 namespace a3 {
@@ -258,7 +259,8 @@
                                                    uint32_t* __restrict__ tile_off, uint32_t n_frames,
                                                    unsigned long long* __restrict__ frame_darts, unsigned long long cap,
                                                    uint32_t* __restrict__ frame_base, PlanWords* __restrict__ plan,
-                                                   uint4* __restrict__ zero_p, uint32_t zero_n16) {
+                                                   uint4* __restrict__ zero_p, uint32_t zero_n16,
+                                                   uint32_t* __restrict__ live_tiles, uint32_t* __restrict__ live_cnt) {
     if (blockIdx.x == n_frames) {
         for (uint32_t i = threadIdx.x; i < zero_n16; i += 256) zero_p[i] = make_uint4(0u, 0u, 0u, 0u);
         __syncthreads();
@@ -266,9 +268,9 @@
         return;
     }
     __shared__ uint32_t s_wave[4];
-    __shared__ uint32_t s_run;
+    __shared__ uint32_t s_run, s_run_live;
     const size_t base = (size_t)(first_frame + blockIdx.x) * tiles;
-    if (threadIdx.x == 0) s_run = 0;
+    if (threadIdx.x == 0) { s_run = 0; s_run_live = 0; }
     __syncthreads();
     for (uint32_t t0 = 0; t0 < tiles; t0 += 256) {
         const uint32_t t = t0 + threadIdx.x;
@@ -283,9 +285,14 @@
         const uint32_t excl = block_excl_scan_256(v, s_wave, &total);
         if (t < tiles) tile_off[base + t] = s_run + excl;
         __syncthreads();
-        if (threadIdx.x == 0) s_run += total;
+        uint32_t total_live;
+        const uint32_t rank = block_excl_scan_256(v ? 1u : 0u, s_wave, &total_live);
+        if (v) live_tiles[base + s_run_live + rank] = t;
         __syncthreads();
-    }
+        if (threadIdx.x == 0) { s_run += total; s_run_live += total_live; }
+        __syncthreads();
+    }
+    if (threadIdx.x == 0) live_cnt[first_frame + blockIdx.x] = s_run_live;
 }
 
 __device__ __forceinline__ uint32_t row3(uint64_t l, uint64_t c, uint64_t r, int i) {
@@ -339,10 +346,12 @@
 
 __global__ __launch_bounds__(256) void k_dart_assign(const uint64_t* __restrict__ bits, int W, int H, uint32_t first_frame,
                                                      const uint32_t* __restrict__ frame_base, const uint32_t* __restrict__ tile_off,
-                                                     uint32_t* __restrict__ pix_base, const uint32_t* __restrict__ tile_darts,
+                                                     uint32_t* __restrict__ pix_base,
                                                      uint64_t* __restrict__ d_rec, uint32_t* __restrict__ d_succ,
                                                      const uint32_t* __restrict__ n_live, int dbg,
-                                                     const unsigned long long* __restrict__ tile_mask, uint32_t tiles, uint32_t n_frames) {
+                                                     const unsigned long long* __restrict__ tile_mask, uint32_t tiles, uint32_t n_frames,
+                                                     const uint32_t* __restrict__ live_tiles, const uint32_t* __restrict__ live_cnt,
+                                                     uint32_t rows, uint32_t* __restrict__ longest) {
     __shared__ uint32_t s_wave[4];
     __shared__ uint64_t s_t[kTileRows + 2][kTileWords + 2];
     __shared__ uint64_t s_nodes[256];
@@ -354,118 +363,135 @@
     __shared__ uint32_t s_multi;
     __shared__ uint16_t s_lut[256];
     const int wpr = (int)words_per_row((uint32_t)W);
-    const uint32_t n_wg = tiles * n_frames, chunk = (n_wg + 7u) >> 3, g = (blockIdx.x & 7u) * chunk + (blockIdx.x >> 3);
-    if (g >= n_wg) return;
-    const uint32_t f = g / tiles, tile = g - f * tiles;
-    if (tile_darts[(size_t)(first_frame + f) * tiles + tile] == 0u) return;
+    const LiveSlot slot = live_slot(blockIdx.x, rows, n_frames);
+    if (slot.f >= n_frames) return;
+    const uint32_t f = slot.f;
+    const size_t fbase = (size_t)(first_frame + f) * tiles;
+    const uint32_t n_list = live_cnt[first_frame + f];
+    uint32_t tile = live_tiles[fbase + slot.r];
+    if (longest && blockIdx.x == 0) {
+        uint32_t m = 0;
+        for (uint32_t i = threadIdx.x; i < n_frames; i += 256) m = max(m, live_cnt[first_frame + i]);
+#pragma unroll
+        for (int o = 32; o > 0; o >>= 1) m = max(m, (uint32_t)__shfl_xor((int)m, o));
+        if ((threadIdx.x & 63u) == 0) s_wave[threadIdx.x >> 6] = m;
+        __syncthreads();
+        if (threadIdx.x == 0) *longest = max(max(s_wave[0], s_wave[1]), max(s_wave[2], s_wave[3]));
+        __syncthreads();
+    }
     if (n_live && *n_live == 0u) return;
-    const uint32_t dart0 = frame_base[f] + tile_off[(size_t)(first_frame + f) * tiles + tile];
-    if (dbg == 1) return;
-    __shared__ uint32_t s_cnt[256];
-    const unsigned long long* tm = tile_mask + ((size_t)(first_frame + f) * tiles + tile) * kCountHalves;
-    static_assert(kCountHalves == 4 && kTileWords == 4 && kTileRows == 64, "four 64-bit word masks per tile, four word columns of 64 rows");
-    unsigned long long cm[4];
-#pragma unroll
-    for (int c = 0; c < 4; c++)
-        cm[c] = ((tm[0] >> (16 * c)) & 0xFFFFull) | (((tm[1] >> (16 * c)) & 0xFFFFull) << 16) | (((tm[2] >> (16 * c)) & 0xFFFFull) << 32) | (((tm[3] >> (16 * c)) & 0xFFFFull) << 48);
-    const unsigned long long m0 = cm[0], m1 = cm[1], m2 = cm[2], m3 = cm[3];
-    tile_stage(bits + (size_t)(first_frame + f) * wpr * H, W, H, tile, s_t);
-    s_cnt[threadIdx.x] = 0;
-    s_mark[threadIdx.x] = 0; s_mark[256 + threadIdx.x] = 0;
-    s_lut[threadIdx.x] = kPixLut.v[threadIdx.x];
-    if (threadIdx.x == 0) s_multi = 0;
-    __syncthreads();
-    const uint32_t a0 = (uint32_t)__popcll(m0), a1 = a0 + (uint32_t)__popcll(m1), a2 = a1 + (uint32_t)__popcll(m2), n_act = a2 + (uint32_t)__popcll(m3);
-    for (uint32_t k = threadIdx.x; k < n_act; k += 256) {
-        const uint32_t part = (k >= a0) + (k >= a1) + (k >= a2);
-        const unsigned long long mm = part == 0 ? m0 : (part == 1 ? m1 : (part == 2 ? m2 : m3));
-        const uint32_t w = part * 64u + (uint32_t)select_bit(mm, k - (part == 0 ? 0u : (part == 1 ? a0 : (part == 2 ? a1 : a2))));
-        const Nb8 nb = tile_nb8(s_t, (int)(w & 63u), (int)(w >> 6));
-        uint64_t p[8];
-        pdart_words(nb, p);
-        uint64_t nodes = 0;
-        uint32_t nd = 0;
-#pragma unroll
-        for (int q = 0; q < 8; q++) { nd += __popcll(p[q]); nodes |= p[q]; }
-        const uint64_t s1 = p[0] ^ p[1] ^ p[2], k1 = (p[0] & p[1]) | (p[2] & (p[0] ^ p[1]));
-        const uint64_t s2 = p[3] ^ p[4] ^ p[5], k2 = (p[3] & p[4]) | (p[5] & (p[3] ^ p[4]));
-        const uint64_t s3 = p[6] ^ p[7], k3 = p[6] & p[7];
-        const uint64_t k4 = (s1 & s2) | (s3 & (s1 ^ s2));
-        const uint64_t t = k1 ^ k2 ^ k3, q1 = (k1 & k2) | (k3 & (k1 ^ k2));
-        s_nodes[w] = nodes;
-        const uint64_t c1 = t ^ k4, c2 = q1 | (t & k4);
-        s_c0[w] = s1 ^ s2 ^ s3; s_c1[w] = c1; s_c2[w] = c2;
-        if ((c1 | c2) != 0ull) s_multi = 1u;
-        s_cnt[w] = nd | ((uint32_t)__popcll(nodes) << 17);
-        s_wofrank[k] = (uint8_t)w; s_rank[w] = (uint8_t)k;
-    }
-    __syncthreads();
-    uint32_t total_p;
-    const uint32_t excl_p = block_excl_scan_256(s_cnt[threadIdx.x], s_wave, &total_p);
-    const uint32_t excl_d = excl_p & 0x1FFFFu, excl_n = excl_p >> 17, total_n = total_p >> 17;
-    s_dbase[threadIdx.x] = excl_d;
-    {
-        const uint32_t cw = s_cnt[threadIdx.x] >> 17;
-        if (cw) {
-            const uint32_t k = s_rank[threadIdx.x];
-            s_nbk[k] = (uint16_t)excl_n;
-            if (excl_n) atomicOr(&s_mark[(excl_n - 1u) >> 5], 1u << ((excl_n - 1u) & 31u));
-            const uint32_t seg = (excl_n + 63u) >> 6;
-            if ((seg << 6) < excl_n + cw) s_fr[seg] = (uint8_t)k;
-        }
-    }
-    if (dbg == 2) return;
-    __syncthreads();
-    if (dbg == 3) return;
-    const int tx = tile % dart_tiles_x((uint32_t)W), ty = tile / dart_tiles_x((uint32_t)W);
-    uint32_t* pbf = pix_base + (size_t)f * W * H;
-    const bool single = __builtin_amdgcn_readfirstlane((int)s_multi) == 0;
-    for (uint32_t n = threadIdx.x; n < total_n; n += 256) {
-        const uint32_t seg = n >> 6;
-        const uint32_t marks_below = __builtin_amdgcn_mbcnt_hi(s_mark[2u * seg + 1u], __builtin_amdgcn_mbcnt_lo(s_mark[2u * seg], 0u));
-        const uint32_t kr = (uint32_t)s_fr[seg] + marks_below;
-        const uint32_t w = s_wofrank[kr], r = n - (uint32_t)s_nbk[kr];
-        const uint64_t m = s_nodes[w];
-        const int i = select_bit(m, r);
-        const int jl = w >> 6, rl = w & 63;
-        const int wj = tx * kTileWords + jl, wy = ty * kTileRows + rl;
-        const uint32_t F = tile_F(s_t, rl, jl, i);
-        const uint32_t lut = s_lut[F];
-        uint32_t P = lut & 0xFFu;
-        const uint64_t below = (1ull << i) - 1ull;
-        const uint32_t off = single ? (uint32_t)__popcll(m & below)
-                                    : (uint32_t)__popcll(s_c0[w] & below) + 2u * (uint32_t)__popcll(s_c1[w] & below) + 4u * (uint32_t)__popcll(s_c2[w] & below);
-        const int x = 64 * wj + i;
-        uint32_t cur = dart0 + s_dbase[w] + off;
-        if ((i == 0 || i == 63 || rl == 0 || rl == kTileRows - 1) && dbg != 4) pbf[(size_t)wy * W + x] = cur;
-        const int kW = x > 0 ? (int)((lut >> 8) & 15u) : 15, kE = x + 1 < W ? (int)(lut >> 12) : 15;
-        const uint32_t xy = (uint32_t)x | ((uint32_t)wy << 16);
-        while (P) {
-            const int k = __ffs(P) - 1;
-            P &= P - 1;
-            const uint32_t info = (uint32_t)k | (k == kW ? kInfoW : 0u) | (k == kE ? kInfoE : 0u);
-            if (dbg != 4) d_rec[cur] = dart_rec(xy, F, info, f);
-            const uint32_t rr = ((F >> k) | (F << (8 - k))) & 0xFFu;
-            const int ko = (k + (31 - __clz(rr))) & 7, kin = (ko + 4) & 7;
-            const int lx = jl * 64 + i + dir_dx(ko), ly = rl + dir_dy(ko);
-            uint32_t succ;
-            if (lx >= 0 && lx < kTileWords * 64 && ly >= 0 && ly < kTileRows) {
-                const int j2 = lx >> 6, i2 = lx & 63, w2 = j2 * kTileRows + ly;
-                const uint32_t P2 = (uint32_t)s_lut[tile_F(s_t, ly, j2, i2)] & 0xFFu;
-                succ = cur;
-                if ((P2 >> kin) & 1u) {
-                    const uint64_t below2 = (1ull << i2) - 1ull;
-                    const uint32_t off2 = single ? (uint32_t)__popcll(s_nodes[w2] & below2)
-                                                 : (uint32_t)__popcll(s_c0[w2] & below2) + 2u * (uint32_t)__popcll(s_c1[w2] & below2) +
-                                                   4u * (uint32_t)__popcll(s_c2[w2] & below2);
-                    succ = dart0 + s_dbase[w2] + off2 + (uint32_t)__popc(P2 & ((1u << kin) - 1u));
+    for (uint32_t r = slot.r; r < n_list; r += rows) {
+        if (r != slot.r) tile = live_tiles[fbase + r];
+        const uint32_t dart0 = frame_base[f] + tile_off[(size_t)(first_frame + f) * tiles + tile];
+        if (dbg == 1) return;
+        __shared__ uint32_t s_cnt[256];
+        const unsigned long long* tm = tile_mask + ((size_t)(first_frame + f) * tiles + tile) * kCountHalves;
+        static_assert(kCountHalves == 4 && kTileWords == 4 && kTileRows == 64, "four 64-bit word masks per tile, four word columns of 64 rows");
+        unsigned long long cm[4];
+#pragma unroll
+        for (int c = 0; c < 4; c++)
+            cm[c] = ((tm[0] >> (16 * c)) & 0xFFFFull) | (((tm[1] >> (16 * c)) & 0xFFFFull) << 16) | (((tm[2] >> (16 * c)) & 0xFFFFull) << 32) | (((tm[3] >> (16 * c)) & 0xFFFFull) << 48);
+        const unsigned long long m0 = cm[0], m1 = cm[1], m2 = cm[2], m3 = cm[3];
+        tile_stage(bits + (size_t)(first_frame + f) * wpr * H, W, H, tile, s_t);
+        s_cnt[threadIdx.x] = 0;
+        s_mark[threadIdx.x] = 0; s_mark[256 + threadIdx.x] = 0;
+        s_lut[threadIdx.x] = kPixLut.v[threadIdx.x];
+        if (threadIdx.x == 0) s_multi = 0;
+        __syncthreads();
+        const uint32_t a0 = (uint32_t)__popcll(m0), a1 = a0 + (uint32_t)__popcll(m1), a2 = a1 + (uint32_t)__popcll(m2), n_act = a2 + (uint32_t)__popcll(m3);
+        for (uint32_t k = threadIdx.x; k < n_act; k += 256) {
+            const uint32_t part = (k >= a0) + (k >= a1) + (k >= a2);
+            const unsigned long long mm = part == 0 ? m0 : (part == 1 ? m1 : (part == 2 ? m2 : m3));
+            const uint32_t w = part * 64u + (uint32_t)select_bit(mm, k - (part == 0 ? 0u : (part == 1 ? a0 : (part == 2 ? a1 : a2))));
+            const Nb8 nb = tile_nb8(s_t, (int)(w & 63u), (int)(w >> 6));
+            uint64_t p[8];
+            pdart_words(nb, p);
+            uint64_t nodes = 0;
+            uint32_t nd = 0;
+#pragma unroll
+            for (int q = 0; q < 8; q++) { nd += __popcll(p[q]); nodes |= p[q]; }
+            const uint64_t s1 = p[0] ^ p[1] ^ p[2], k1 = (p[0] & p[1]) | (p[2] & (p[0] ^ p[1]));
+            const uint64_t s2 = p[3] ^ p[4] ^ p[5], k2 = (p[3] & p[4]) | (p[5] & (p[3] ^ p[4]));
+            const uint64_t s3 = p[6] ^ p[7], k3 = p[6] & p[7];
+            const uint64_t k4 = (s1 & s2) | (s3 & (s1 ^ s2));
+            const uint64_t t = k1 ^ k2 ^ k3, q1 = (k1 & k2) | (k3 & (k1 ^ k2));
+            s_nodes[w] = nodes;
+            const uint64_t c1 = t ^ k4, c2 = q1 | (t & k4);
+            s_c0[w] = s1 ^ s2 ^ s3; s_c1[w] = c1; s_c2[w] = c2;
+            if ((c1 | c2) != 0ull) s_multi = 1u;
+            s_cnt[w] = nd | ((uint32_t)__popcll(nodes) << 17);
+            s_wofrank[k] = (uint8_t)w; s_rank[w] = (uint8_t)k;
+        }
+        __syncthreads();
+        uint32_t total_p;
+        const uint32_t excl_p = block_excl_scan_256(s_cnt[threadIdx.x], s_wave, &total_p);
+        const uint32_t excl_d = excl_p & 0x1FFFFu, excl_n = excl_p >> 17, total_n = total_p >> 17;
+        s_dbase[threadIdx.x] = excl_d;
+        {
+            const uint32_t cw = s_cnt[threadIdx.x] >> 17;
+            if (cw) {
+                const uint32_t k = s_rank[threadIdx.x];
+                s_nbk[k] = (uint16_t)excl_n;
+                if (excl_n) atomicOr(&s_mark[(excl_n - 1u) >> 5], 1u << ((excl_n - 1u) & 31u));
+                const uint32_t seg = (excl_n + 63u) >> 6;
+                if ((seg << 6) < excl_n + cw) s_fr[seg] = (uint8_t)k;
+            }
+        }
+        if (dbg == 2) return;
+        __syncthreads();
+        if (dbg == 3) return;
+        const int tx = tile % dart_tiles_x((uint32_t)W), ty = tile / dart_tiles_x((uint32_t)W);
+        uint32_t* pbf = pix_base + (size_t)f * W * H;
+        const bool single = __builtin_amdgcn_readfirstlane((int)s_multi) == 0;
+        for (uint32_t n = threadIdx.x; n < total_n; n += 256) {
+            const uint32_t seg = n >> 6;
+            const uint32_t marks_below = __builtin_amdgcn_mbcnt_hi(s_mark[2u * seg + 1u], __builtin_amdgcn_mbcnt_lo(s_mark[2u * seg], 0u));
+            const uint32_t kr = (uint32_t)s_fr[seg] + marks_below;
+            const uint32_t w = s_wofrank[kr], r = n - (uint32_t)s_nbk[kr];
+            const uint64_t m = s_nodes[w];
+            const int i = select_bit(m, r);
+            const int jl = w >> 6, rl = w & 63;
+            const int wj = tx * kTileWords + jl, wy = ty * kTileRows + rl;
+            const uint32_t F = tile_F(s_t, rl, jl, i);
+            const uint32_t lut = s_lut[F];
+            uint32_t P = lut & 0xFFu;
+            const uint64_t below = (1ull << i) - 1ull;
+            const uint32_t off = single ? (uint32_t)__popcll(m & below)
+                                        : (uint32_t)__popcll(s_c0[w] & below) + 2u * (uint32_t)__popcll(s_c1[w] & below) + 4u * (uint32_t)__popcll(s_c2[w] & below);
+            const int x = 64 * wj + i;
+            uint32_t cur = dart0 + s_dbase[w] + off;
+            if ((i == 0 || i == 63 || rl == 0 || rl == kTileRows - 1) && dbg != 4) pbf[(size_t)wy * W + x] = cur;
+            const int kW = x > 0 ? (int)((lut >> 8) & 15u) : 15, kE = x + 1 < W ? (int)(lut >> 12) : 15;
+            const uint32_t xy = (uint32_t)x | ((uint32_t)wy << 16);
+            while (P) {
+                const int k = __ffs(P) - 1;
+                P &= P - 1;
+                const uint32_t info = (uint32_t)k | (k == kW ? kInfoW : 0u) | (k == kE ? kInfoE : 0u);
+                if (dbg != 4) d_rec[cur] = dart_rec(xy, F, info, f);
+                const uint32_t rr = ((F >> k) | (F << (8 - k))) & 0xFFu;
+                const int ko = (k + (31 - __clz(rr))) & 7, kin = (ko + 4) & 7;
+                const int lx = jl * 64 + i + dir_dx(ko), ly = rl + dir_dy(ko);
+                uint32_t succ;
+                if (lx >= 0 && lx < kTileWords * 64 && ly >= 0 && ly < kTileRows) {
+                    const int j2 = lx >> 6, i2 = lx & 63, w2 = j2 * kTileRows + ly;
+                    const uint32_t P2 = (uint32_t)s_lut[tile_F(s_t, ly, j2, i2)] & 0xFFu;
+                    succ = cur;
+                    if ((P2 >> kin) & 1u) {
+                        const uint64_t below2 = (1ull << i2) - 1ull;
+                        const uint32_t off2 = single ? (uint32_t)__popcll(s_nodes[w2] & below2)
+                                                     : (uint32_t)__popcll(s_c0[w2] & below2) + 2u * (uint32_t)__popcll(s_c1[w2] & below2) +
+                                                       4u * (uint32_t)__popcll(s_c2[w2] & below2);
+                        succ = dart0 + s_dbase[w2] + off2 + (uint32_t)__popc(P2 & ((1u << kin) - 1u));
+                    }
+                } else {
+                    succ = kNone;
                 }
-            } else {
-                succ = kNone;
+                if (dbg != 4 || succ == 0x12345678u) d_succ[cur] = succ;
+                cur++;
             }
-            if (dbg != 4 || succ == 0x12345678u) d_succ[cur] = succ;
-            cur++;
-        }
+        }
+        if (r + rows >= n_list) break;
+        __syncthreads();
     }
 }
 
@@ -1516,7 +1542,8 @@
 
 static size_t tile_off_offset(uint32_t W, uint32_t H, uint32_t n_frames) { return (size_t)dart_tiles(W, H) * n_frames; }
 static size_t tile_mask_offset_bytes(uint32_t W, uint32_t H, uint32_t n_frames) { return ((size_t)dart_tiles(W, H) * n_frames * 4 * (1 + kCountHalves) + 7) & ~(size_t)7; }
-size_t tile_darts_bytes(uint32_t W, uint32_t H, uint32_t n_frames) { return tile_mask_offset_bytes(W, H, n_frames) + (size_t)dart_tiles(W, H) * n_frames * kCountHalves * 8; }
+static size_t live_tiles_offset_bytes(uint32_t W, uint32_t H, uint32_t n_frames) { return tile_mask_offset_bytes(W, H, n_frames) + (size_t)dart_tiles(W, H) * n_frames * kCountHalves * 8; }
+size_t tile_darts_bytes(uint32_t W, uint32_t H, uint32_t n_frames) { return live_tiles_offset_bytes(W, H, n_frames) + ((size_t)dart_tiles(W, H) + 1) * n_frames * 4; }
 
 hipError_t launch_dart_count(hipStream_t st, const DartCountLaunch& d) {
     const uint64_t* const bits = d.bits; const int W = d.W, H = d.H; const uint32_t first_frame = d.first_frame, n_frames = d.n_frames;
@@ -1530,9 +1557,10 @@
     else
         hipLaunchKernelGGL(k_dart_count<64>, dim3(((wpr + kCountLanes - 1) / kCountLanes) * tiles_y, n_frames, kCountHalves), dim3(64), 0, st, bits, W, H, first_frame,
                            frame_darts, tile_darts, h1, tmask);
+    uint32_t* live = reinterpret_cast<uint32_t*>(reinterpret_cast<uint8_t*>(tile_darts) + live_tiles_offset_bytes((uint32_t)W, (uint32_t)H, n_frames));
     hipLaunchKernelGGL(k_tile_scan, dim3(n_frames + (plan ? 1u : 0u)), dim3(256), 0, st, tile_darts, h1, tiles_x * tiles_y, first_frame,
                        tile_darts + (size_t)tiles_x * tiles_y * n_frames, n_frames, frame_darts, (unsigned long long)d.plan_cap, d.frame_base, plan,
-                       reinterpret_cast<uint4*>(d.zero_p), (uint32_t)(d.zero_bytes / 16));
+                       reinterpret_cast<uint4*>(d.zero_p), (uint32_t)(d.zero_bytes / 16), live, live + (size_t)tiles_x * tiles_y * n_frames);
     return hipGetLastError();
 }
 
@@ -1541,8 +1569,12 @@
     const uint32_t* const tile_off = c.tile_darts + tile_off_offset((uint32_t)c.W, (uint32_t)c.H, c.batch_frames);
     const unsigned long long* const tile_mask = reinterpret_cast<const unsigned long long*>(
         reinterpret_cast<const uint8_t*>(c.tile_darts) + tile_mask_offset_bytes((uint32_t)c.W, (uint32_t)c.H, c.batch_frames));
-    hipLaunchKernelGGL(k_dart_assign, dim3((tiles * c.n_frames + 7u) / 8u * 8u), dim3(256), 0, st, c.bits, c.W, c.H, c.first_frame, c.frame_base, tile_off,
-                       c.pix_base, c.tile_darts, c.d_rec, c.d_succ, c.n_live, c.dbg, tile_mask, tiles, c.n_frames);
+    const uint32_t* const live = reinterpret_cast<const uint32_t*>(
+        reinterpret_cast<const uint8_t*>(c.tile_darts) + live_tiles_offset_bytes((uint32_t)c.W, (uint32_t)c.H, c.batch_frames));
+    const uint32_t rows = assign_rows(c.assign_rows, tiles);
+    hipLaunchKernelGGL(k_dart_assign, dim3(assign_grid(rows, c.n_frames)), dim3(256), 0, st, c.bits, c.W, c.H, c.first_frame, c.frame_base, tile_off,
+                       c.pix_base, c.d_rec, c.d_succ, c.n_live, c.dbg, tile_mask, tiles, c.n_frames, live,
+                       live + (size_t)tiles * c.batch_frames, rows, c.n_frames <= kLiveMaxFrames ? c.longest_list : nullptr);
     if (c.dbg && c.dbg != 5) return hipGetLastError();
     hipLaunchKernelGGL(k_dart_link, dim3(blocks_for(c.n_darts, 256, 4096)), dim3(256), 0, st, c.W, c.H, c.first_frame, c.pix_base, c.bits, c.d_rec, c.d_succ,
                        c.n_darts, c.n_live);
```
